# geo-ant/varpro

Measured on AMD Instinct MI355X. Metric: independent fits/sec (double-exp, m=1024, fp64), higher is better.
Workload: dtype f64; 1 GPU; B=65536 fits/GPU, m=1024, fp64, double-exp+offset (n=3, q=2), one full LM fit per step; batch_per_gpu=65536, m=1024, batches_in_flight=2, world_size=1, parallelism=batch-sharded x1

## Files before the change

bindings/rust/varpro_hip.rs:

```rust
#![allow(non_camel_case_types)]
use std::ffi::{c_char, c_void, CStr};
use std::ptr::null_mut;

use levenberg_marquardt::LeastSquaresProblem;
use nalgebra::storage::Owned;
use nalgebra::{DMatrix, DVector, Dyn};
use varpro::model::SeparableNonlinearModel;

#[repr(C)]
#[derive(Clone, Copy)]
pub struct vp_model_desc {
    pub n_basis: i32,
    pub n_params: i32,
    pub kind: [i32; 8],
    pub param: [[i32; 2]; 8],
}
#[repr(C)]
#[derive(Clone, Copy)]
pub struct vp_lm_opts {
    pub ftol: f64,
    pub xtol: f64,
    pub gtol: f64,
    pub stepbound: f64,
    pub patience: i32,
    pub scale_diag: i32,
}
#[repr(C)]
#[derive(Clone, Copy, Default)]
pub struct vp_report {
    pub termination: i32,
    pub n_evals: i32,
    pub objective: f64,
}
pub enum vp_batch {}

pub const VP_BASIS_CONST: i32 = 0;
pub const VP_BASIS_EXP_DECAY: i32 = 1;
pub const VP_BASIS_EXP_RATE: i32 = 2;
pub const VP_BASIS_EXP_COS: i32 = 3;
pub const VP_BASIS_SIN_PHASE: i32 = 4;
pub const VP_F64: i32 = 0;
pub const VP_FLAG_OWN_STREAM: i32 = 8;
pub const VP_FLAG_NO_GRID_RECURRENCE: i32 = 16;

#[link(name = "varpro_hip")]
extern "C" {
    pub fn vp_batch_create(h: *mut *mut vp_batch, model: *const vp_model_desc, dtype: i32, m: i64, s: i64, b: i64,
        t: *const c_void, y: *const c_void, w: *const c_void, svd_epsilon: f64, flags: i32, device: i32,
        hip_stream: *mut c_void) -> i32;
    pub fn vp_batch_destroy(h: *mut vp_batch);
    pub fn vp_set_params(h: *mut vp_batch, alpha: *const c_void) -> i32;
    pub fn vp_params(h: *mut vp_batch, alpha_out: *mut c_void) -> i32;
    pub fn vp_residuals(h: *mut vp_batch, r_out: *mut c_void, status: *mut i32) -> i32;
    pub fn vp_jacobian(h: *mut vp_batch, j_out: *mut c_void, status: *mut i32) -> i32;
    pub fn vp_linear_coeffs(h: *mut vp_batch, c_out: *mut c_void, status: *mut i32) -> i32;
    pub fn vp_weighted_data(h: *mut vp_batch, yw_out: *mut c_void) -> i32;
    pub fn vp_set_observations(h: *mut vp_batch, y: *const c_void) -> i32;
    pub fn vp_cost(h: *mut vp_batch, cost_out: *mut f64) -> i32;
    pub fn vp_evaluate(h: *mut vp_batch, alpha: *const c_void, r: *mut c_void, j: *mut c_void, c: *mut c_void,
        cost: *mut f64, status: *mut i32) -> i32;
    pub fn vp_basis(h: *mut vp_batch, alpha: *const c_void, phi: *mut c_void, dphi: *mut c_void, flags: i32) -> i32;
    pub fn vp_lm_opts_default(o: *mut vp_lm_opts, dtype: i32);
    pub fn vp_fit(h: *mut vp_batch, opts: *const vp_lm_opts, alpha_inout: *mut c_void, c_out: *mut c_void,
        rep: *mut vp_report) -> i32;
    pub fn vp_best_fit(h: *mut vp_batch, fit_out: *mut c_void) -> i32;
    pub fn vp_debug_gram_evaluate(h: *mut vp_batch, alpha: *const c_void, out: *mut f64) -> i32;
    pub fn vp_summary(h: *mut vp_batch, out: *mut f64) -> i32;
    pub fn vp_summary_device(h: *mut vp_batch, dev_out4: *mut f64) -> i32;
    pub fn vp_global_fit_condition(h: *mut vp_batch, cond_out: *mut f64) -> i32;
    pub fn vp_fit_trace(h: *mut vp_batch, opts: *const vp_lm_opts, alpha_inout: *mut c_void, c_out: *mut c_void,
        rep: *mut vp_report, trace_out: *mut f64, trace_rows: i32) -> i32;
    pub fn vp_statistics(h: *mut vp_batch, cov_out: *mut c_void, chi2_out: *mut f64, sigma_out: *mut c_void,
        status: *mut i32) -> i32;
    pub fn vp_global_statistics(h: *mut vp_batch, cov_alpha_out: *mut c_void, chi2_out: *mut f64, coef_cov_out: *mut c_void,
        coef_alpha_cov_out: *mut c_void, sigma_out: *mut c_void, status: *mut i32) -> i32;
    pub fn vp_set_rhs_allreduce(h: *mut vp_batch,
        f: Option<extern "C" fn(*mut c_void, i64, *mut c_void, *mut c_void) -> i32>, user: *mut c_void,
        global_rhs_count: i64) -> i32;
    pub fn vp_set_fit_kernel(h: *mut vp_batch, which: i32) -> i32;
    pub fn vp_set_timing(h: *mut vp_batch, enable: i32) -> i32;
    pub fn vp_last_kernel_ms(h: *mut vp_batch, which: i32, ms: *mut f32) -> i32;
    pub fn vp_synchronize(h: *mut vp_batch) -> i32;
    pub fn vp_last_error_detail() -> i32;
    pub fn vp_version() -> *const c_char;
    pub fn vp_device_count() -> i32;
    pub fn vp_last_error() -> *const c_char;
}

fn last_error() -> String {
    unsafe { CStr::from_ptr(vp_last_error()).to_string_lossy().into_owned() }
}

pub struct GpuSeparableProblem {
    h: *mut vp_batch,
    m: usize,
    s: usize,
    n: usize,
    q: usize,
    alpha: DVector<f64>,
}

impl GpuSeparableProblem {
    pub fn build(desc: vp_model_desc, x: &DVector<f64>, y: &DMatrix<f64>, w: Option<&DVector<f64>>, eps: Option<f64>,
                 initial: DVector<f64>) -> Result<Self, String> {
        let (m, s) = (y.nrows(), y.ncols());
        let mut h: *mut vp_batch = null_mut();
        let rc = unsafe {
            vp_batch_create(&mut h, &desc, VP_F64, m as i64, s as i64, 1, x.as_ptr() as *const c_void,
                y.as_ptr() as *const c_void, w.map_or(std::ptr::null(), |w| w.as_ptr() as *const c_void),
                eps.unwrap_or(-1.0), VP_FLAG_OWN_STREAM, 0, null_mut())
        };
        if rc != 0 { return Err(last_error()); }
        let mut p = Self { h, m, s, n: desc.n_basis as usize, q: desc.n_params as usize, alpha: initial.clone() };
        p.set_params(&initial);
        Ok(p)
    }
    pub fn linear_coefficients(&self) -> Option<DMatrix<f64>> {
// ... 155 lines not shown
```

include/varpro_hip.h:

```cpp
#ifndef VARPRO_HIP_H
#define VARPRO_HIP_H

#include <stdint.h>

#ifdef __cplusplus
extern "C" {
#endif

#define VP_MAX_BASIS 8
#define VP_MAX_PARAMS 8
#define VP_MAX_BASIS_PARAMS 2
#define VP_MAX_PAIRS 16

enum { VP_F64 = 0, VP_F32 = 1 };

enum {
    VP_BASIS_CONST = 0,
    VP_BASIS_EXP_DECAY = 1,
    VP_BASIS_EXP_RATE = 2,
    VP_BASIS_EXP_COS = 3,
    VP_BASIS_SIN_PHASE = 4,
    VP_BASIS_EXTERNAL = 5
};

// ... 70 lines not shown
typedef struct vp_batch vp_batch;


int vp_batch_create(vp_batch **h, const vp_model_desc *model, int dtype, int64_t m, int64_t S, int64_t B,
                    const void *t, const void *Y, const void *w, double svd_epsilon, int flags, int device,
                    void *hip_stream);

void vp_batch_destroy(vp_batch *h);


int vp_set_params(vp_batch *h, const void *alpha);

int vp_params(vp_batch *h, void *alpha_out);

int vp_residuals(vp_batch *h, void *r_out, int32_t *status);

int vp_jacobian(vp_batch *h, void *J_out, int32_t *status);

int vp_linear_coeffs(vp_batch *h, void *C_out, int32_t *status);

int vp_weighted_data(vp_batch *h, void *Yw_out);

int vp_set_observations(vp_batch *h, const void *Y);

int vp_cost(vp_batch *h, double *cost_out);

int vp_evaluate(vp_batch *h, const void *alpha, void *r_out, void *J_out, void *C_out, double *cost_out,
                int32_t *status);


enum { VP_BASIS_SKIP_INVARIANT = 1 };
int vp_basis(vp_batch *h, const void *alpha, void *Phi_out, void *dPhi_out, int flags);

int vp_batch_create_external(vp_batch **h, int32_t n_basis, int32_t n_params, int32_t n_pairs, const int32_t *pair_basis,
                             const int32_t *pair_param, int dtype, int64_t m, int64_t S, int64_t B, const void *Y,
                             const void *w, double svd_epsilon, int flags, int device, void *hip_stream);
int vp_set_params_with_basis(vp_batch *h, const void *alpha, const void *Phi, const void *dPhi);
int vp_jacobian_with_derivatives(vp_batch *h, const void *dPhi, void *J_out, int32_t *status);
int vp_evaluate_with_basis(vp_batch *h, const void *alpha, const void *Phi, const void *dPhi, void *r_out, void *J_out,
                           void *C_out, double *cost_out, int32_t *status);


void vp_lm_opts_default(vp_lm_opts *opts, int dtype);

enum { VP_FIT_DERIVATIVES_ON_ACCEPT = 1 };
enum { VP_WANT_BASIS = 1, VP_WANT_DERIVATIVES = 2 };
int vp_fit_begin(vp_batch *h, const vp_lm_opts *opts, const void *alpha0, int flags);
int vp_fit_step_with_basis(vp_batch *h, const void *Phi, const void *dPhi, void *alpha_trial_out, int32_t *want_out,
                           int64_t *n_active_out);
int vp_fit_end(vp_batch *h, void *alpha_out, void *C_out, vp_report *rep);
int vp_fit_active_set(vp_batch *h, int32_t *index_out, int32_t *count_out);

int vp_fit(vp_batch *h, const vp_lm_opts *opts, void *alpha_inout, void *C_out, vp_report *rep);

int vp_fit_trace(vp_batch *h, const vp_lm_opts *opts, void *alpha_inout, void *C_out, vp_report *rep,
                 double *trace_out, int trace_rows);

int vp_best_fit(vp_batch *h, void *fit_out);

int vp_statistics(vp_batch *h, void *cov_out, double *reduced_chi2_out, void *conf_sigma_out, int32_t *status);

int vp_global_statistics(vp_batch *h, void *cov_alpha_out, double *reduced_chi2_out, void *coef_cov_out,
                         void *coef_alpha_cov_out, void *conf_sigma_out, int32_t *status);

int vp_summary(vp_batch *h, double out[4]);

int vp_global_fit_condition(vp_batch *h, double *cond_out);

int vp_summary_device(vp_batch *h, double *dev_out4);

int vp_reduce_cost(vp_batch *h, void *rccl_comm, double out[4]);

typedef int (*vp_allreduce_fn)(void *dev_doubles, int64_t count, void *hip_stream, void *user);
int vp_set_rhs_allreduce(vp_batch *h, vp_allreduce_fn fn, void *user, int64_t global_rhs_count);

enum { VP_FIT_KERNEL_AUTO = 0, VP_FIT_KERNEL_WAVE = 1, VP_FIT_KERNEL_SLOTS = 2 };
int vp_set_fit_kernel(vp_batch *h, int which);


enum { VP_KERNEL_EVALUATE = 0, VP_KERNEL_BASIS = 1, VP_KERNEL_FIT = 2 };
int vp_set_timing(vp_batch *h, int enable);
int vp_last_kernel_ms(vp_batch *h, int which, float *ms);

int vp_synchronize(vp_batch *h);
const char *vp_last_error(void);
int vp_last_error_detail(void);
const char *vp_version(void);
int vp_device_count(void);

#ifdef __cplusplus
}
#endif
#endif
```

varpro_amd/_lib.py:

```python
import ctypes as C
import os

try:
    import torch
except Exception:
    torch = None

VP_MAX_BASIS = 8
VP_MAX_PARAMS = 8
VP_MAX_BASIS_PARAMS = 2
VP_MAX_PAIRS = 16

VP_F64, VP_F32 = 0, 1
VP_FLAG_DEVICE_PTRS, VP_FLAG_T_PER_PROBLEM, VP_FLAG_W_PER_PROBLEM, VP_FLAG_OWN_STREAM = 1, 2, 4, 8
VP_FLAG_NO_GRID_RECURRENCE = 16
VP_FLAG_STREAM_ROWS = 32
VP_BASIS_SKIP_INVARIANT = 1
VP_FIT_DERIVATIVES_ON_ACCEPT = 1
VP_WANT_BASIS, VP_WANT_DERIVATIVES = 1, 2
VP_KERNEL_EVALUATE, VP_KERNEL_BASIS, VP_KERNEL_FIT = 0, 1, 2
VP_ST_OK, VP_ST_NONFINITE, VP_ST_NOT_EVALUATED = 0, 1, 2

VP_ERR_OK, VP_ERR_INVALID, VP_ERR_UNSUPPORTED, VP_ERR_HIP, VP_ERR_NO_DEVICE = 0, -1, -2, -3, -4

_HERE = os.path.dirname(os.path.abspath(__file__))
LIB_PATH = os.path.join(_HERE, "lib", "libvarpro_hip.so")
if os.environ.get("VARPRO_HIP_LIBRARY"):
    LIB_PATH = os.path.abspath(os.environ["VARPRO_HIP_LIBRARY"])

ALLREDUCE_FN = C.CFUNCTYPE(C.c_int, C.c_void_p, C.c_int64, C.c_void_p, C.c_void_p)

VP_FIT_KERNEL_AUTO, VP_FIT_KERNEL_WAVE, VP_FIT_KERNEL_SLOTS = 0, 1, 2

ABI_SYMBOLS = [
    "vp_batch_create", "vp_batch_destroy", "vp_set_params", "vp_params", "vp_residuals", "vp_jacobian",
    "vp_linear_coeffs", "vp_weighted_data", "vp_set_observations", "vp_cost", "vp_evaluate", "vp_basis", "vp_lm_opts_default", "vp_fit", "vp_fit_trace",
    "vp_best_fit", "vp_statistics", "vp_summary", "vp_summary_device", "vp_global_fit_condition", "vp_set_rhs_allreduce", "vp_set_fit_kernel", "vp_set_timing", "vp_last_kernel_ms", "vp_synchronize", "vp_last_error",
    "vp_last_error_detail", "vp_version", "vp_device_count",
    "vp_batch_create_external", "vp_set_params_with_basis", "vp_jacobian_with_derivatives", "vp_evaluate_with_basis",
    "vp_reduce_cost", "vp_fit_begin", "vp_fit_step_with_basis", "vp_fit_end", "vp_fit_active_set", "vp_global_statistics",
]


DEBUG_SYMBOLS = ["vp_debug_gram_evaluate", "vp_debug_lmpar_gram", "vp_debug_set_refit"]


class VarproHipUnavailable(ImportError):
    pass


class VarproHipError(RuntimeError):
    def __init__(self, code, message, detail=0):
        super().__init__("varpro_hip error %d: %s" % (code, message))
        self.code = code
        self.detail = detail


class ModelDesc(C.Structure):
    _fields_ = [
        ("n_basis", C.c_int32),
        ("n_params", C.c_int32),
        ("kind", C.c_int32 * VP_MAX_BASIS),
        ("param", (C.c_int32 * VP_MAX_BASIS_PARAMS) * VP_MAX_BASIS),
    ]


class LmOpts(C.Structure):
    _fields_ = [
        ("ftol", C.c_double),
        ("xtol", C.c_double),
        ("gtol", C.c_double),
        ("stepbound", C.c_double),
        ("patience", C.c_int32),
        ("scale_diag", C.c_int32),
    ]


class Report(C.Structure):
    _fields_ = [("termination", C.c_int32), ("n_evals", C.c_int32), ("objective", C.c_double)]


_lib = None


def load():
    global _lib
    if _lib is not None:
        return _lib
    if not os.path.exists(LIB_PATH):
        raise VarproHipUnavailable(
            "%s not found: build it with `python -c 'import __graft_entry__ as g; g.build()'` "
            "(or `make -C varpro_amd/csrc`). varpro_amd has no CPU fallback." % LIB_PATH)
    try:
        lib = C.CDLL(LIB_PATH)
    except OSError as e:
        raise VarproHipUnavailable("cannot load %s: %s" % (LIB_PATH, e))
    vp, i32p, dp = C.c_void_p, C.POINTER(C.c_int32), C.POINTER(C.c_double)
    lib.vp_batch_create.argtypes = [C.POINTER(vp), C.POINTER(ModelDesc), C.c_int, C.c_int64, C.c_int64, C.c_int64,
                                    vp, vp, vp, C.c_double, C.c_int, C.c_int, vp]
    lib.vp_batch_create_external.argtypes = [C.POINTER(vp), C.c_int32, C.c_int32, C.c_int32, i32p, i32p, C.c_int, C.c_int64,
                                             C.c_int64, C.c_int64, vp, vp, C.c_double, C.c_int, C.c_int, vp]
    lib.vp_set_params_with_basis.argtypes = [vp, vp, vp, vp]
    lib.vp_jacobian_with_derivatives.argtypes = [vp, vp, vp, vp]
    lib.vp_evaluate_with_basis.argtypes = [vp, vp, vp, vp, vp, vp, vp, vp, vp]
    lib.vp_fit_begin.argtypes = [vp, C.POINTER(LmOpts), vp, C.c_int]
    lib.vp_fit_step_with_basis.argtypes = [vp, vp, vp, vp, vp, C.POINTER(C.c_int64)]
    lib.vp_fit_end.argtypes = [vp, vp, vp, vp]
    lib.vp_fit_active_set.argtypes = [vp, vp, vp]
    lib.vp_batch_destroy.argtypes = [vp]
    lib.vp_batch_destroy.restype = None
    lib.vp_set_params.argtypes = [vp, vp]
    lib.vp_set_observations.argtypes = [vp, vp]
    lib.vp_params.argtypes = [vp, vp]
    lib.vp_residuals.argtypes = [vp, vp, vp]
    lib.vp_jacobian.argtypes = [vp, vp, vp]
    lib.vp_linear_coeffs.argtypes = [vp, vp, vp]
    lib.vp_weighted_data.argtypes = [vp, vp]
    lib.vp_cost.argtypes = [vp, vp]
    lib.vp_evaluate.argtypes = [vp, vp, vp, vp, vp, vp, vp]
    lib.vp_basis.argtypes = [vp, vp, vp, vp, C.c_int]
    lib.vp_lm_opts_default.argtypes = [C.POINTER(LmOpts), C.c_int]
    lib.vp_lm_opts_default.restype = None
    lib.vp_fit.argtypes = [vp, C.POINTER(LmOpts), vp, vp, vp]
    lib.vp_fit_trace.argtypes = [vp, C.POINTER(LmOpts), vp, vp, vp, vp, C.c_int]
    lib.vp_best_fit.argtypes = [vp, vp]
    lib.vp_debug_gram_evaluate.argtypes = [vp, vp, vp]
    lib.vp_debug_lmpar_gram.argtypes = [C.c_int64, C.c_int, vp, vp, vp, vp, vp, vp, vp]
    lib.vp_debug_set_refit.argtypes = [vp, C.c_int]
    lib.vp_statistics.argtypes = [vp, vp, vp, vp, vp]
    lib.vp_global_statistics.argtypes = [vp, vp, vp, vp, vp, vp, vp]
    lib.vp_summary.argtypes = [vp, dp]
    lib.vp_summary_device.argtypes = [vp, vp]
    lib.vp_global_fit_condition.argtypes = [vp, vp]
    lib.vp_reduce_cost.argtypes = [vp, vp, dp]
    lib.vp_set_rhs_allreduce.argtypes = [vp, ALLREDUCE_FN, vp, C.c_int64]
    lib.vp_set_fit_kernel.argtypes = [vp, C.c_int]
    lib.vp_set_timing.argtypes = [vp, C.c_int]
    lib.vp_last_kernel_ms.argtypes = [vp, C.c_int, C.POINTER(C.c_float)]
    lib.vp_synchronize.argtypes = [vp]
    lib.vp_last_error.restype = C.c_char_p
    lib.vp_last_error_detail.restype = C.c_int
    lib.vp_version.restype = C.c_char_p
    lib.vp_device_count.restype = C.c_int
    _ = i32p
    _lib = lib
    return lib


def check(rc):
    if rc != 0:
        lib = load()
        raise VarproHipError(rc, lib.vp_last_error().decode("utf-8", "replace"), lib.vp_last_error_detail())


def device_count():
    return load().vp_device_count()
```

varpro_amd/batch.py:

```python
import ctypes as C

import numpy as np

from . import _lib
from ._lib import check

try:
    import torch
except Exception:
    torch = None

REPORT_DTYPE = np.dtype([("termination", np.int32), ("n_evals", np.int32), ("objective", np.float64)])

STATUS_OK, STATUS_NONFINITE, STATUS_NOT_EVALUATED = 0, 1, 2


def _is_torch(a):
    return torch is not None and isinstance(a, torch.Tensor)


class LevenbergMarquardt:

    def __init__(self, dtype=np.float64):
        eps = float(np.finfo(dtype).eps)
# ... 274 lines not shown
        J = self._empty((self.B, self.q, self.S * self.m))
        st = self._empty((self.B,), np.int32)
        check(self.lib.vp_jacobian(self._h, self._ptr(J), self._ptr(st)))
        if not self._have_params:
            J = None
        return (J, st) if with_status else J

    @_device_entry
    def linear_coefficients(self):
        Cm = self._empty((self.B, self.S, self.n))
        check(self.lib.vp_linear_coeffs(self._h, self._ptr(Cm), None))
        return Cm.reshape(self.B, self.n) if self.single_rhs else Cm

    @_device_entry
    def weighted_data(self):
        Yw = self._empty((self.B, self.S, self.m))
        check(self.lib.vp_weighted_data(self._h, self._ptr(Yw)))
        return Yw.reshape(self.B, self.m) if self.single_rhs else Yw

    @_device_entry
    def cost(self):
        c = self._empty((self.B,), np.float64)
        check(self.lib.vp_cost(self._h, self._ptr(c)))
        return c

    @_device_entry
    def evaluate(self, alpha, want_residuals=True, want_jacobian=True):
        a = self._as_array(alpha).reshape(self.B, self.q)
        r = self._empty((self.B, self.S * self.m)) if want_residuals else None
        J = self._empty((self.B, self.q, self.S * self.m)) if want_jacobian else None
        Cm = self._empty((self.B, self.S, self.n))
        cost = self._empty((self.B,), np.float64)
        st = self._empty((self.B,), np.int32)
        check(self.lib.vp_evaluate(self._h, self._ptr(a), self._ptr(r), self._ptr(J), self._ptr(Cm), self._ptr(cost),
                                   self._ptr(st)))
        self._have_params = True
        return dict(r=r, J=J, C=Cm.reshape(self.B, self.n) if self.single_rhs else Cm, cost=cost, status=st)

    @_device_entry
    def basis(self, alpha, skip_invariant=False, want_phi=True, want_dphi=True, out_phi=None, out_dphi=None):
        a = self._as_array(alpha).reshape(self.B, self.q)
        ncols = self.n - (sum(1 for k in self.model.kinds if k == 0) if skip_invariant else 0)
        phi = out_phi if out_phi is not None else (self._empty((self.B, ncols, self.m)) if want_phi else None)
        dphi = out_dphi if out_dphi is not None else (self._empty((self.B, self.p, self.m)) if want_dphi else None)
        check(self.lib.vp_basis(self._h, self._ptr(a), self._ptr(phi), self._ptr(dphi),
                                _lib.VP_BASIS_SKIP_INVARIANT if skip_invariant else 0))
        return phi, dphi

    @_device_entry
    def fit(self, alpha0, solver=None, want_coefficients=True):
        solver = solver or LevenbergMarquardt(self.np_dtype)
        opts = solver._c()
        a = self._as_array(alpha0).reshape(self.B, self.q)
        a = a.clone() if _is_torch(a) else a.copy()
        Cm = self._empty((self.B, self.S, self.n)) if want_coefficients else None
        if self.device_mode:
            rep_t = torch.empty((self.B, 16), dtype=torch.uint8, device=self._torch_device())
            check(self.lib.vp_fit(self._h, C.byref(opts), self._ptr(a), self._ptr(Cm), self._ptr(rep_t)))
            self._have_params = True
            rep = rep_t
            if Cm is not None and self.single_rhs:
                Cm = Cm.reshape(self.B, self.n)
            return a, Cm, rep
        else:
            rep = np.zeros(self.B, dtype=REPORT_DTYPE)
            check(self.lib.vp_fit(self._h, C.byref(opts), self._ptr(a), self._ptr(Cm), C.c_void_p(rep.ctypes.data)))
            self._have_params = True
        if Cm is not None and self.single_rhs:
            Cm = Cm.reshape(self.B, self.n)
        return a, Cm, rep

    @_device_entry
    def fit_begin(self, alpha0, solver=None, derivatives_on_accept=False):
        solver = solver or LevenbergMarquardt(self.np_dtype)
        opts = solver._c()
        a = self._as_array(alpha0).reshape(self.B, self.q)
        flags = _lib.VP_FIT_DERIVATIVES_ON_ACCEPT if derivatives_on_accept else 0
        check(self.lib.vp_fit_begin(self._h, C.byref(opts), self._ptr(a), flags))
        self._have_params = False
        self._xf_trial = self._empty((self.B, self.q))
        self._xf_want = self._empty((self.B,), np.int32)

    @_device_entry
    def fit_step_with_basis(self, Phi, dPhi=None, want_count=True):
        Phi = self._as_array(Phi).reshape(self.B, self.n, self.m)
        dPhi = None if dPhi is None else self._as_array(dPhi).reshape(self.B, self.p, self.m)
        self._ext_keep = (Phi, dPhi)
        nact = C.c_int64(0)
        check(self.lib.vp_fit_step_with_basis(self._h, self._ptr(Phi), self._ptr(dPhi), self._ptr(self._xf_trial),
                                              self._ptr(self._xf_want), C.byref(nact) if want_count else None))
        return self._xf_trial, self._xf_want, (int(nact.value) if want_count else None)

    @_device_entry
    def fit_active_set(self, index_out=None, count_out=None):
        idx = index_out if index_out is not None else self._empty((self.B,), np.int32)
        cnt = count_out if count_out is not None else self._empty((1,), np.int32)
        check(self.lib.vp_fit_active_set(self._h, self._ptr(idx), self._ptr(cnt)))
        return idx, cnt

    @_device_entry
    def fit_end(self, want_coefficients=True):
        a = self._empty((self.B, self.q))
        Cm = self._empty((self.B, self.n) if self.single_rhs else (self.B, self.S, self.n)) if want_coefficients else None
        if self.device_mode:
            rep = torch.empty((self.B, 16), dtype=torch.uint8, device=self._torch_device())
            check(self.lib.vp_fit_end(self._h, self._ptr(a), self._ptr(Cm), self._ptr(rep)))
        else:
            rep = np.zeros(self.B, dtype=REPORT_DTYPE)
            check(self.lib.vp_fit_end(self._h, self._ptr(a), self._ptr(Cm), C.c_void_p(rep.ctypes.data)))
        self._have_params = True
        return a, Cm, rep

    def fit_with_model(self, evaluate, alpha0, solver=None, derivatives_on_accept=False, max_steps=None, check_every=1):
        self.fit_begin(alpha0, solver, derivatives_on_accept)
        solver = solver or LevenbergMarquardt(self.np_dtype)
        limit = max_steps if max_steps is not None else 2 * (solver.patience * (self.q + 1) + 2)
        alpha, want = self._as_array(alpha0).reshape(self.B, self.q), None
# ... 156 lines not shown
```

varpro_amd/cpp/varpro.hpp:

```cpp
#pragma once
#include <algorithm>
#include <cmath>
#include <cstdint>
#include <functional>
#include <map>
#include <memory>
#include <optional>
#include <stdexcept>
#include <string>
#include <utility>
#include <vector>

#include "../../include/varpro_hip.h"

namespace varpro {

enum class Basis : int32_t {
    Const = VP_BASIS_CONST,
    ExpDecay = VP_BASIS_EXP_DECAY,
    ExpRate = VP_BASIS_EXP_RATE,
    ExpCos = VP_BASIS_EXP_COS,
    SinPhase = VP_BASIS_SIN_PHASE
};
inline int arity(Basis k) {
// ... 238 lines not shown
        n = model.desc.n_basis;
        q = model.desc.n_params;
        if ((int64_t)Y.size() != B * S * m) throw std::invalid_argument("Y must hold B*S*m values");
        check(vp_batch_create(&h_, &model.desc, VP_F64, m, S, B, model.x.data(), Y.data(), weights ? weights->data() : nullptr,
                              epsilon, VP_FLAG_OWN_STREAM, device, nullptr));
    }
    BatchProblem(const BatchProblem &) = delete;
    BatchProblem &operator=(const BatchProblem &) = delete;
    BatchProblem(BatchProblem &&o) noexcept { *this = std::move(o); }
    BatchProblem &operator=(BatchProblem &&o) noexcept {
        std::swap(h_, o.h_);
        m = o.m, S = o.S, B = o.B, n = o.n, q = o.q;
        return *this;
    }
    ~BatchProblem() {
        if (h_) vp_batch_destroy(h_);
    }
    vp_batch *handle() const { return h_; }
    void set_params(const std::vector<double> &alpha) { check(vp_set_params(h_, alpha.data())); }
    void set_observations(const std::vector<double> &Y) {
        if ((int64_t)Y.size() != B * S * m) throw std::invalid_argument("Y must hold B*S*m values");
        check(vp_set_observations(h_, Y.data()));
    }
    std::vector<int32_t> status() const {
        std::vector<int32_t> st((size_t)B);
        check(vp_linear_coeffs(h_, nullptr, st.data()));
        return st;
    }
    std::vector<double> residuals() const {
        std::vector<double> r((size_t)(B * S * m));
        check(vp_residuals(h_, r.data(), nullptr));
        return r;
    }
    std::vector<double> jacobian() const {
        std::vector<double> J((size_t)(B * q * S * m));
        check(vp_jacobian(h_, J.data(), nullptr));
        return J;
    }
    std::vector<double> linear_coefficients() const {
        std::vector<double> C((size_t)(B * S * n));
        check(vp_linear_coeffs(h_, C.data(), nullptr));
        return C;
    }
    std::vector<double> best_fit() const {
        std::vector<double> f((size_t)(B * S * m));
        check(vp_best_fit(h_, f.data()));
        return f;
    }
    std::vector<vp_report> fit(std::vector<double> &alpha_inout, const LevenbergMarquardt &solver = LevenbergMarquardt()) {
        std::vector<vp_report> rep((size_t)B);
        check(vp_fit(h_, &solver.o, alpha_inout.data(), nullptr, rep.data()));
        return rep;
    }
    struct Statistics {
        std::vector<double> covariance;
        std::vector<double> reduced_chi2;
        std::vector<double> conf_sigma;
        std::vector<int32_t> status;
        int64_t m = 0, dof = 0;
        std::vector<double> confidence_band_radius(int64_t b, double probability) const {
            if (!(probability > 0.0 && probability < 1.0)) throw std::invalid_argument("probability must be in (0,1)");
            const double tq = student_t_quantile(0.5 * (1.0 + probability), (double)dof);
            std::vector<double> r((size_t)m);
            for (int64_t i = 0; i < m; ++i) r[(size_t)i] = tq * conf_sigma[(size_t)(b * m + i)];
            return r;
        }
    };
    Statistics statistics() const {
        Statistics s;
        const size_t k = (size_t)(n + q);
        s.covariance.resize((size_t)B * k * k);
        s.reduced_chi2.resize((size_t)B);
        s.conf_sigma.resize((size_t)(B * m));
        s.status.resize((size_t)B);
        s.m = m;
        s.dof = m - (int64_t)k;
        check(vp_statistics(h_, s.covariance.data(), s.reduced_chi2.data(), s.conf_sigma.data(), s.status.data()));
        return s;
    }
    struct GlobalStatistics {
        std::vector<double> cov_alpha;
        std::vector<double> reduced_chi2;
        std::vector<double> coef_cov;
        std::vector<double> coef_alpha_cov;
        std::vector<double> conf_sigma;
        std::vector<int32_t> status;
        int64_t m = 0, S = 1, dof = 0;
        std::vector<double> confidence_band_radius(int64_t b, int64_t s, double probability) const {
            if (!(probability > 0.0 && probability < 1.0)) throw std::invalid_argument("probability must be in (0,1)");
            if (conf_sigma.empty()) throw std::logic_error("global_statistics(true) computes the band");
            const double tq = student_t_quantile(0.5 * (1.0 + probability), (double)dof);
            std::vector<double> r((size_t)m);
            for (int64_t i = 0; i < m; ++i) r[(size_t)i] = tq * conf_sigma[(size_t)((b * S + s) * m + i)];
            return r;
        }
    };
    GlobalStatistics global_statistics(bool want_confidence_sigma = false) const {
        GlobalStatistics g;
        g.cov_alpha.resize((size_t)(B * q * q));
        g.reduced_chi2.resize((size_t)B);
        g.coef_cov.resize((size_t)(B * S * n * n));
        g.coef_alpha_cov.resize((size_t)(B * S * n * q));
        if (want_confidence_sigma) g.conf_sigma.resize((size_t)(B * S * m));
        g.status.resize((size_t)B);
        g.m = m;
        g.S = S;
// ... 300 lines not shown
```

varpro_amd/csrc/vp_api.hip:

```cpp
#include <hip/hip_runtime.h>

#include <dlfcn.h>

#include <cfloat>
#include <cmath>
#include <cstdio>
#include <cstdlib>
#include <cstring>
#include <string>

#include "../../include/varpro_hip.h"
#include "../../include/varpro_hip_debug.h"
#include "vp_registry.hpp"
#include "vp_extfit_api.hpp"
#include "vp_mrhs.hpp"
#include "vp_gstats.hpp"

using namespace vp;

#ifndef VP_MRHS_EXACT_AFTER
#define VP_MRHS_EXACT_AFTER 8
#endif

namespace {
// ... 18 lines not shown

template <typename T>
__global__ void weight_data_kernel(const T *Y, const T *__restrict__ w, T *Yw, int m, int64_t cols_per_problem,
                                   int64_t w_stride, int64_t total) {
    for (int64_t idx = blockIdx.x * (int64_t)blockDim.x + threadIdx.x; idx < total;
         idx += (int64_t)gridDim.x * blockDim.x) {
        const int64_t col = idx / m;
        const int i = (int)(idx - col * m);
        const int64_t b = col / cols_per_problem;
        Yw[idx] = w ? (T)(w[b * w_stride + i] * Y[idx]) : Y[idx];
    }
}

__global__ void reduce_rhs_kernel(const double *__restrict__ cost_bs, const int32_t *__restrict__ status_bs,
                                  double *__restrict__ cost_b, int32_t *__restrict__ status_b, int S, int64_t B) {
    const int64_t b = blockIdx.x;
    if (b >= B) return;
    double acc = 0.0;
    int st = 0;
    for (int s0 = threadIdx.x; s0 < S; s0 += 8 * blockDim.x) {
        double c[8];
        int v[8];
#pragma unroll
        for (int k = 0; k < 8; ++k) {
            const int s = s0 + k * (int)blockDim.x;
            const bool in = s < S;
            c[k] = in ? cost_bs[b * S + s] : 0.0;
            v[k] = in ? status_bs[b * S + s] : 0;
        }
#pragma unroll
        for (int k = 0; k < 8; ++k) {
            acc += c[k];
            st = v[k] > st ? v[k] : st;
        }
    }
    __shared__ double sh[1024];
    __shared__ int shs[1024];
    sh[threadIdx.x] = acc;
    shs[threadIdx.x] = st;
    __syncthreads();
    for (int off = blockDim.x / 2; off > 0; off >>= 1) {
        if ((int)threadIdx.x < off) {
            sh[threadIdx.x] += sh[threadIdx.x + off];
            shs[threadIdx.x] = shs[threadIdx.x] > shs[threadIdx.x + off] ? shs[threadIdx.x] : shs[threadIdx.x + off];
        }
        __syncthreads();
    }
    if (threadIdx.x == 0) {
        if (cost_b) cost_b[b] = sh[0];
        if (status_b) status_b[b] = shs[0];
    }
}

__global__ void summary_kernel(const vp_report *__restrict__ rep, int64_t B, double *__restrict__ out4) {
    double c = 0, ok = 0, bad = 0, ev = 0;
    for (int64_t b = blockIdx.x * (int64_t)blockDim.x + threadIdx.x; b < B; b += (int64_t)gridDim.x * blockDim.x) {
        const vp_report r = rep[b];
        if (r.objective == r.objective) c += r.objective;
        if (r.termination > 0) ok += 1.0;
        else bad += 1.0;
        ev += (double)r.n_evals;
    }
    __shared__ double sh[4][256];
    sh[0][threadIdx.x] = c;
    sh[1][threadIdx.x] = ok;
    sh[2][threadIdx.x] = bad;
    sh[3][threadIdx.x] = ev;
    __syncthreads();
    for (int off = blockDim.x / 2; off > 0; off >>= 1) {
        if ((int)threadIdx.x < off)
            for (int k = 0; k < 4; ++k) sh[k][threadIdx.x] += sh[k][threadIdx.x + off];
        __syncthreads();
    }
    if (threadIdx.x == 0)
        for (int k = 0; k < 4; ++k) atomicAdd(&out4[k], sh[k][0]);
}

__global__ void mrhs_reduce_partials_kernel(const double *part, int gx, int nacc, int64_t B, double *tot) {
    const int64_t idx = blockIdx.x * (int64_t)blockDim.x + threadIdx.x;
    if (idx >= B * nacc) return;
    const int64_t b = idx / nacc;
    const int i = (int)(idx - b * nacc);
    double s = 0.0;
    for (int g = 0; g < gx; ++g) s += part[((size_t)b * nacc + i) * gx + g];
    tot[idx] = s;
}

template <typename T> __global__ void grid_check_kernel(const T *t, int m, int64_t ngrids, int *flag) {
    const int64_t g = blockIdx.x;
    if (g >= ngrids) return;
    const T *tg = t + g * (int64_t)m;
    const double t0 = (double)tg[0];
    const double dt = ((double)tg[m - 1] - t0) / (double)(m - 1);
    const double tol = 4.0 * (sizeof(T) == 8 ? 2.220446049250313e-16 : 1.1920928955078125e-07);
    bool ok = (dt == dt) && (dt - dt == 0.0) && dt != 0.0;
    for (int i = threadIdx.x; i < m; i += blockDim.x) {
        const double lat = __builtin_fma((double)i, dt, t0);
        const double dev = __builtin_fabs((double)tg[i] - lat);
        if (!(dev <= tol * __builtin_fabs((double)tg[i] - t0))) ok = false;
    }
    if (!ok) atomicAnd(flag, 0);
}

}

struct vp_batch {
    vp_model_desc model;
    int dtype;
    int64_t m, S, B;
    int n, q, p;
    int flags;
    int device;
    double eps;
    hipStream_t stream;
    bool own_stream;
    const KernelEntry *kern;
    void *d_t, *d_w, *d_yw;
    void *d_alpha;
    void *d_C;
    void *d_R;
    double *d_cost_bs;
    int32_t *d_status_bs;
    double *d_cost;
    int32_t *d_status;
    vp_report *d_report;
    double *d_sum4;
    bool grid_uniform;
    bool have_params;
    bool r_valid;
    bool have_report;
    bool timing;
    hipEvent_t ev0, ev1;
    float last_ms[3];
    bool have_mrhs;
    MrhsWs mrhs;
    vp_allreduce_fn rhs_allreduce;
    void *rhs_allreduce_user;
    int64_t rhs_global;
    double *d_mrhs_tot;
    void *d_gen_lm;
    int32_t *d_gen_nactive;
    int fit_kernel;
    int *d_queue;
    int num_cus;
    void *tmp_a, *tmp_b;
    void *d_gen_ws;
    int gen_blocks;
    int64_t m_user;
    hipGraphExec_t mrhs_graph;
    hipGraphExec_t mrhs_graph_tail;
    bool external;
    int ext_np;
    int32_t ext_pb[VP_MAX_PAIRS], ext_pp[VP_MAX_PAIRS];
    const void *ext_phi, *ext_dphi;
    void *ext_phi_own, *ext_dphi_own;
    int mrhs_graph_len;
    int mrhs_graph_iters;
    int mrhs_prev_nfev;
    int mrhs_same_count;
    int32_t *h_nactive;
    int32_t *h_nactive_dev;
    MrhsIo *h_io;
    MrhsIo *h_io_dev;
    vp_lm_opts mrhs_graph_opts;
    hipStream_t cap_stream;
    bool mrhs_graph_failed;
    void *d_xf_state;
    void *d_xf_trial;
    int32_t *d_xf_want;
    void *d_xf_ctrial;
    int32_t *d_xf_active;
    int64_t xf_known_active;
    int32_t *d_xf_nactive;
    int32_t *h_xf_nactive;
    bool xf_running;
    bool xf_init;
    int xf_flags;
    int64_t xf_steps;
    vp_lm_opts xf_opts;
    int32_t *d_rescue;
    void *d_rescue_ws;
    int rescue_slot;
    bool rescue_off;
};

namespace {

bool device_ptrs(const vp_batch *h) { return (h->flags & VP_FLAG_DEVICE_PTRS) != 0; }

struct InBuf {
    const void *dptr = nullptr;
    void *tmp = nullptr;
    int init(vp_batch *h, const void *user, size_t bytes) {
        if (!user) {
            dptr = nullptr;
// ... 206 lines not shown
    return 0;
}

int run_evaluate(vp_batch *h, void *r_dev, void *J_dev, void *C_dev) {
    if (h->external && !h->ext_phi)
        return fail(VP_ERR_INVALID, "the columns of the handle's current parameters are not known (after vp_fit_end: call "
                                    "vp_set_params_with_basis with Phi / dPhi at the fitted parameters first)");
    if (h->external && !h->d_gen_ws &&
        !external_resident(h->dtype, h->n, h->ext_np, h->m, h->m_user ? h->m_user : h->m, J_dev != nullptr))
        if (int rc = ensure_gen_ws(h)) return rc;
    LaunchParams p;
    fill_params(h, p);
    p.r_out = r_dev;
    p.J_out = J_dev;
    p.C_out = C_dev;
    p.cost_out = h->d_cost_bs;
    p.status = h->d_status_bs;
    Timer tm(h, VP_KERNEL_EVALUATE);
    int rc;
    if (h->have_mrhs) {
        p.mrhs_ws = &h->mrhs;
        p.mrhs_mode = 1;
        rc = h->kern->mrhs_factor(p);
        if (rc == VP_ERR_OK) rc = h->kern->mrhs_stream(p);
    } else {
        rc = h->kern->evaluate(p);
    }
    tm.stop();
    if (rc != VP_ERR_OK) return fail(rc, "evaluate kernel launch failed");
    return reduce_rhs(h);
}

struct DeviceGuard {
    int prev = -1;
    bool armed = false;
    int enter(int device) {
        if (hipGetDevice(&prev) != hipSuccess) prev = -1;
        if (prev != device) {
            VP_HIP(hipSetDevice(device));
            armed = prev >= 0;
        }
        return 0;
    }
    ~DeviceGuard() {
        if (armed) (void)hipSetDevice(prev);
    }
};

#define VP_ENTER(h)                                                                                                   \
    if (!(h)) return fail(VP_ERR_INVALID, "null handle");                                                             \
    DeviceGuard dev_guard__;                                                                                          \
    if (int rc__ = dev_guard__.enter((h)->device)) return rc__

int mrhs_fit(vp_batch *h, const vp_lm_opts *opts, void *alpha_inout, void *C_out, vp_report *rep, double *trace_out,
             int trace_rows) {
    if (!h->have_mrhs && !h->kern->mrhs_fit_whole) return fail(VP_ERR_UNSUPPORTED, "no MRHS kernels for this (model, m)");
    vp_lm_opts o;
    if (opts) o = *opts;
    else vp_lm_opts_default(&o, h->dtype);
    const size_t ts = tsize(h->dtype);
    const hipMemcpyKind kin = device_ptrs(h) ? hipMemcpyDeviceToDevice : hipMemcpyHostToDevice;
    const bool use_io = device_ptrs(h) && h->have_mrhs;
    if (!h->h_nactive) {
        VP_HIP(hipHostMalloc((void **)&h->h_nactive, 2 * sizeof(int32_t), hipHostMallocMapped));
        VP_HIP(hipHostGetDevicePointer((void **)&h->h_nactive_dev, h->h_nactive, 0));
        VP_HIP(hipHostMalloc((void **)&h->h_io, sizeof(MrhsIo), hipHostMallocMapped));
        VP_HIP(hipHostGetDevicePointer((void **)&h->h_io_dev, h->h_io, 0));
        std::memset(h->h_io, 0, sizeof(MrhsIo));
    }
    if (use_io) {
        h->h_io->alpha_in = alpha_inout;
        h->h_io->alpha_out = alpha_inout;
        h->h_io->C_out = C_out;
        h->h_io->rep_out = rep;
    } else {
        std::memset(h->h_io, 0, sizeof(MrhsIo));
        VP_HIP(hipMemcpyAsync(h->d_alpha, alpha_inout, (size_t)h->B * h->q * ts, kin, h->stream));
    }
    LaunchParams p;
    fill_params(h, p);
    p.mrhs_ws = &h->mrhs;
    p.opts = &o;
    OutBuf tr;
    const size_t tr_bytes = (size_t)h->B * (size_t)(trace_rows > 0 ? trace_rows : 0) * (h->q + 4) * sizeof(double);
    if (trace_out && trace_rows > 0) {
        if (int rc = tr.init(h, trace_out, tr_bytes)) return rc;
        VP_HIP(hipMemsetAsync(tr.dptr, 0xFF, tr_bytes, h->stream));
        p.trace = (double *)tr.dptr;
        p.trace_rows = trace_rows;
    }
    if (!h->have_mrhs) {
        p.alpha_out = h->d_alpha;
        p.C_out = h->d_C;
        p.cost_out = h->d_cost_bs;
        p.status = h->d_status_bs;
        p.report = h->d_report;
        if (h->rhs_allreduce) {
            const int nacc = 2 + h->q * h->q + h->q;
            if (!h->d_gen_lm) VP_HIP(hipMalloc(&h->d_gen_lm, (size_t)h->B * h->kern->mrhs_state_bytes));
            if (!h->d_mrhs_tot) VP_HIP(hipMalloc((void **)&h->d_mrhs_tot, (size_t)h->B * nacc * sizeof(double)));
            if (!h->d_gen_nactive) VP_HIP(hipMalloc((void **)&h->d_gen_nactive, sizeof(int32_t)));
            VP_HIP(hipMemsetAsync(h->d_gen_nactive, 0, sizeof(int32_t), h->stream));
            p.gen_lm_state = h->d_gen_lm;
            p.gen_acc = h->d_mrhs_tot;
            p.gen_nactive = h->d_gen_nactive;
            p.mrhs_S_global = h->rhs_global;
            Timer tm(h, VP_KERNEL_FIT);
            p.gen_phase = 1;
            if (int rc = h->kern->mrhs_fit_whole(p)) return fail(rc, "generic global-fit (init) launch failed");
            const int max_iter = o.patience * (h->q + 1) + 2;
            for (int it = 0; it < max_iter; ++it) {
                p.gen_phase = 2;
                if (int rc = h->kern->mrhs_fit_whole(p)) return fail(rc, "generic global-fit (sums) launch failed");
                if (h->rhs_allreduce(h->d_mrhs_tot, h->B * nacc, (void *)h->stream, h->rhs_allreduce_user) != 0)
                    return fail(VP_ERR_INVALID, "the right-hand-side all-reduce callback reported an error");
                p.gen_phase = 3;
                if (int rc = h->kern->mrhs_fit_whole(p)) return fail(rc, "generic global-fit (step) launch failed");
                if ((it & 3) == 3 || it + 1 == max_iter) {
                    int32_t nact = 0;
                    VP_HIP(hipMemcpyAsync(&nact, h->d_gen_nactive, sizeof(int32_t), hipMemcpyDeviceToHost, h->stream));
                    VP_HIP(hipStreamSynchronize(h->stream));
                    if (nact <= 0) break;
                }
            }
            p.gen_phase = 4;
            if (int rc = h->kern->mrhs_fit_whole(p)) return fail(rc, "generic global-fit (results) launch failed");
            tm.stop();
        } else {
            Timer tm(h, VP_KERNEL_FIT);
            if (int rc = h->kern->mrhs_fit_whole(p)) return fail(rc, "generic global-fit launch failed");
// ... 409 lines not shown
    if (try_uniform) {
        const int one = 1;
        VP_TRY(hipMalloc((void **)&d_gflag, sizeof(int)));
        VP_TRY(hipMemcpyAsync(d_gflag, &one, sizeof(int), hipMemcpyHostToDevice, h->stream));
        const int64_t ngrids = (flags & VP_FLAG_T_PER_PROBLEM) ? B : 1;
        if (dtype == VP_F64)
            hipLaunchKernelGGL(grid_check_kernel<double>, dim3((unsigned)ngrids), dim3(256), 0, h->stream,
                               (const double *)h->d_t, (int)m, ngrids, d_gflag);
        else
            hipLaunchKernelGGL(grid_check_kernel<float>, dim3((unsigned)ngrids), dim3(256), 0, h->stream,
                               (const float *)h->d_t, (int)m, ngrids, d_gflag);
        VP_TRY(hipGetLastError());
    }
    VP_TRY(hipMalloc(&h->d_yw, y_elems * ts));
    {
        void *&ytmp = h->tmp_b;
        const void *ysrc = Y;
        if (!data_on_device) {
            VP_TRY(hipMalloc(&ytmp, y_elems * ts));
            VP_TRY(hipMemcpyAsync(ytmp, Y, y_elems * ts, hipMemcpyHostToDevice, h->stream));
            ysrc = ytmp;
        }
        const int64_t total = (int64_t)y_elems;
        const unsigned grid = (unsigned)std::min<int64_t>((total + 255) / 256, 65536);
        const int64_t wstride = (flags & VP_FLAG_W_PER_PROBLEM) ? m : 0;
        if (dtype == VP_F64)
            hipLaunchKernelGGL(weight_data_kernel<double>, dim3(grid), dim3(256), 0, h->stream, (const double *)ysrc,
                               (const double *)h->d_w, (double *)h->d_yw, (int)m, S, wstride, total);
        else
            hipLaunchKernelGGL(weight_data_kernel<float>, dim3(grid), dim3(256), 0, h->stream, (const float *)ysrc,
                               (const float *)h->d_w, (float *)h->d_yw, (int)m, S, wstride, total);
        VP_TRY(hipGetLastError());
        int gflag = 0;
        if (d_gflag) VP_TRY(hipMemcpyAsync(&gflag, d_gflag, sizeof(int), hipMemcpyDeviceToHost, h->stream));
        VP_TRY(hipStreamSynchronize(h->stream));
        (void)hipFree(ytmp);
        ytmp = nullptr;
        (void)hipFree(d_gflag);
        d_gflag = nullptr;
        h->grid_uniform = gflag != 0;
    }
    VP_TRY(hipMalloc(&h->d_alpha, (size_t)std::max<int64_t>(1, B * h->q) * ts));
    VP_TRY(hipMalloc(&h->d_C, (size_t)B * S * h->n * ts));
    VP_TRY(hipMalloc((void **)&h->d_cost_bs, (size_t)B * S * sizeof(double)));
    VP_TRY(hipMalloc((void **)&h->d_status_bs, (size_t)B * S * sizeof(int32_t)));
    if (S == 1) {
        h->d_cost = h->d_cost_bs;
        h->d_status = h->d_status_bs;
    } else {
        VP_TRY(hipMalloc((void **)&h->d_cost, (size_t)B * sizeof(double)));
        VP_TRY(hipMalloc((void **)&h->d_status, (size_t)B * sizeof(int32_t)));
    }
    VP_TRY(hipMalloc((void **)&h->d_report, (size_t)B * sizeof(vp_report)));
    VP_TRY(hipMalloc((void **)&h->d_sum4, 4 * sizeof(double)));
    VP_TRY(hipMalloc((void **)&h->d_queue, sizeof(int)));
    if (kern->uses_gen_ws && !ext) {
        if (int rc = ensure_gen_ws(h)) {
            vp_batch_destroy(h);
            return rc;
        }
    }
    VP_TRY(hipEventCreate(&h->ev0));
    VP_TRY(hipEventCreate(&h->ev1));
    if (S > 1 && kern->mrhs_factor && kern->mrhs_stream && kern->mrhs_lm && kern->mrhs_finish) {
        const int n_ = h->n, p_ = h->p, q_ = h->q;
        VP_TRY(hipMalloc(&h->mrhs.qthin, (size_t)B * n_ * m * ts));
        VP_TRY(hipMalloc(&h->mrhs.g, (size_t)B * std::max(1, p_) * m * ts));
        VP_TRY(hipMalloc((void **)&h->mrhs.small, (size_t)B * mrhs_small_stride_rt(n_, p_) * sizeof(double)));
        VP_TRY(hipMalloc((void **)&h->mrhs.statusA, (size_t)B * sizeof(int32_t)));
        const int gx_acc = mrhs_gx(S, kern->mrhs_gx_cap > 0 ? kern->mrhs_gx_cap : 256);
        if (gx_acc > VP_MRHS_GX_MAX) {
            vp_batch_destroy(h);
            return fail(VP_ERR_INVALID, "internal: partial-sum slots per problem exceed VP_MRHS_GX_MAX");
        }
        VP_TRY(hipMalloc((void **)&h->mrhs.acc, (size_t)B * gx_acc * (1 + n_ * n_ + p_) * sizeof(double)));
        VP_TRY(hipMalloc(&h->mrhs.lm_state, (size_t)B * kern->mrhs_state_bytes));
        VP_TRY(hipMalloc((void **)&h->mrhs.nactive, 2 * sizeof(int32_t)));
        VP_TRY(hipMalloc((void **)&h->mrhs.done, (size_t)B * sizeof(int32_t)));
        VP_TRY(hipMemsetAsync(h->mrhs.done, 0, (size_t)B * sizeof(int32_t), h->stream));
        VP_TRY(hipMalloc(&h->mrhs.alpha_trial, (size_t)std::max<int64_t>(1, B * q_) * ts));
        for (int i = 0; i < 2; ++i) {
            VP_TRY(hipMalloc(&h->mrhs.cbuf[i], (size_t)B * S * n_ * ts));
            VP_TRY(hipMalloc((void **)&h->mrhs.costbuf[i], (size_t)B * S * sizeof(double)));
            VP_TRY(hipMalloc((void **)&h->mrhs.stbuf[i], (size_t)B * S * sizeof(int32_t)));
        }
        VP_TRY(hipMalloc((void **)&h->mrhs.widx, (size_t)B * sizeof(int32_t)));
        VP_TRY(hipMalloc((void **)&h->mrhs.bidx, (size_t)B * sizeof(int32_t)));
        VP_TRY(hipMalloc((void **)&h->mrhs.jcond, (size_t)B * sizeof(double)));
        VP_TRY(hipMemsetAsync(h->mrhs.jcond, 0, (size_t)B * sizeof(double), h->stream));
        h->have_mrhs = true;
    }
#undef VP_TRY
    for (int k = 0; k < 3; ++k) h->last_ms[k] = -1.f;
    *out = h;
    return VP_ERR_OK;
}

void vp_batch_destroy(vp_batch *h) {
    if (!h) return;
    DeviceGuard dev_guard__;
    (void)dev_guard__.enter(h->device);
    (void)hipStreamSynchronize(h->stream);
    (void)hipFree(h->d_mrhs_tot);
    (void)hipFree(h->d_gen_lm);
    (void)hipFree(h->d_gen_nactive);
    (void)hipFree(h->d_t);
    (void)hipFree(h->d_w);
    (void)hipFree(h->d_yw);
// ... 398 lines not shown
    return copy_out(h, cost_out, h->d_cost, (size_t)h->B * sizeof(double));
}

int vp_evaluate(vp_batch *h, const void *alpha, void *r_out, void *J_out, void *C_out, double *cost_out,
                int32_t *status) {
    VP_ENTER(h);
    VP_NOT_EXTERNAL(h, "vp_evaluate");
    if (!alpha) return fail(VP_ERR_INVALID, "null alpha");
    const size_t ts = tsize(h->dtype);
    VP_HIP(hipMemcpyAsync(h->d_alpha, alpha, (size_t)h->B * h->q * ts,
                          device_ptrs(h) ? hipMemcpyDeviceToDevice : hipMemcpyHostToDevice, h->stream));
    RowOut r, J;
    if (int rc = r.init(h, r_out, (size_t)h->B * h->S)) return rc;
    if (int rc = J.init(h, J_out, (size_t)h->B * h->q * h->S)) return rc;
    if (int rc = run_evaluate(h, r.dptr, J.dptr, h->d_C)) return rc;
    h->have_params = true;
    h->r_valid = false;
    if (int rc = r.finish(h)) return rc;
    if (int rc = J.finish(h)) return rc;
    if (int rc = copy_out(h, C_out, h->d_C, (size_t)h->B * h->S * h->n * ts)) return rc;
    if (int rc = copy_out(h, cost_out, h->d_cost, (size_t)h->B * sizeof(double))) return rc;
    return copy_status(h, status);
}

int vp_basis(vp_batch *h, const void *alpha, void *Phi_out, void *dPhi_out, int flags) {
    VP_ENTER(h);
    VP_NOT_EXTERNAL(h, "vp_basis");
    if (!alpha) return fail(VP_ERR_INVALID, "null alpha");
    const size_t ts = tsize(h->dtype);
    int ncols = 0;
    for (int j = 0; j < h->n; ++j)
        if (!((flags & VP_BASIS_SKIP_INVARIANT) && h->model.kind[j] == VP_BASIS_CONST)) ++ncols;
    InBuf a;
    if (int rc = a.init(h, alpha, (size_t)h->B * h->q * ts)) return rc;
    RowOut phi, dphi;
    if (int rc = phi.init(h, Phi_out, (size_t)h->B * ncols)) return rc;
    if (int rc = dphi.init(h, dPhi_out, (size_t)h->B * h->p)) return rc;
    LaunchParams p;
    fill_params(h, p);
    p.alpha = a.dptr;
    p.Phi_out = phi.dptr;
    p.dPhi_out = dphi.dptr;
    p.basis_flags = flags;
    Timer tm(h, VP_KERNEL_BASIS);
    int rc = h->kern->basis(p);
    tm.stop();
    if (rc != VP_ERR_OK) return fail(rc, "basis kernel launch failed");
    if (int rc2 = phi.finish(h)) return rc2;
    if (int rc2 = dphi.finish(h)) return rc2;
    if (!device_ptrs(h)) VP_HIP(hipStreamSynchronize(h->stream));
    return VP_ERR_OK;
}

int vp_fit(vp_batch *h, const vp_lm_opts *opts, void *alpha_inout, void *C_out, vp_report *rep) {
    return vp_fit_trace(h, opts, alpha_inout, C_out, rep, nullptr, 0);
}

namespace {
constexpr int kRescueBlocks = 8;
int rescue_prepare(vp_batch *h, LaunchParams &p) {
    if (h->rescue_off || h->kern->family == FAMILY_GENERIC || h->kern->gram_fit) return 0;
    if (!h->d_rescue) {
        VP_HIP(hipMalloc((void **)&h->d_rescue, (size_t)(2 + h->B) * sizeof(int32_t)));
        VP_HIP(hipMemsetAsync(h->d_rescue, 0, 2 * sizeof(int32_t), h->stream));
        h->rescue_slot = 0;
    }
    if (!h->d_rescue_ws) {
        const size_t slot = (size_t)(h->n + 1 + h->p + h->q) * (size_t)h->m * tsize(h->dtype);
        VP_HIP(hipMalloc(&h->d_rescue_ws, (size_t)kRescueBlocks * slot));
    }
    p.rescue = h->d_rescue;
    p.rescue_slot = h->rescue_slot;
    return 0;
}
int rescue_refit(vp_batch *h, const LaunchParams &fit_params) {
    if (!fit_params.rescue) return 0;
    LaunchParams p = fit_params;
    p.gen_list_first = 0;
    if (launch_fn fast = find_fit_rescue(h->kern->fit_single)) {
        const int rc = fast(p);
        if (rc == VP_ERR_OK) p.gen_list_first = kFitRescueGrid;
        else if (rc != VP_ERR_UNSUPPORTED) return rc;
    }
    p.rescue = nullptr;
    p.gen_ws = h->d_rescue_ws;
    p.gen_blocks = kRescueBlocks;
    p.gen_list = h->d_rescue;
    p.gen_list_slot = h->rescue_slot;
    p.gen_scale_cols = 1;
    h->rescue_slot ^= 1;
    return generic_kernels(h->dtype)->fit_single(p);
}
}

int vp_fit_trace(vp_batch *h, const vp_lm_opts *opts, void *alpha_inout, void *C_out, vp_report *rep,
                 double *trace_out, int trace_rows) {
    VP_ENTER(h);
    VP_NOT_EXTERNAL(h, "vp_fit");
    if (!alpha_inout) return fail(VP_ERR_INVALID, "null alpha");
    if (h->m_user && (int64_t)h->q > h->m_user * h->S) {
        const size_t ts = tsize(h->dtype);
        VP_HIP(hipMemcpyAsync(h->d_alpha, alpha_inout, (size_t)h->B * h->q * ts,
                              device_ptrs(h) ? hipMemcpyDeviceToDevice : hipMemcpyHostToDevice, h->stream));
        if (int rc = run_evaluate(h, nullptr, nullptr, h->d_C)) return rc;
        OutBuf trw;
        if (trace_out && trace_rows > 0) {
            const size_t trb = (size_t)h->B * (size_t)trace_rows * (h->q + 4) * sizeof(double);
            if (int rc = trw.init(h, trace_out, trb)) return rc;
            VP_HIP(hipMemsetAsync(trw.dptr, 0xFF, trb, h->stream));
        }
        hipLaunchKernelGGL(wrong_dimensions_report_kernel, dim3((unsigned)((h->B + 255) / 256)), dim3(256), 0, h->stream,
                           (const double *)h->d_cost, (const int32_t *)h->d_status, h->B, h->d_report,
                           trw.dptr ? (double *)trw.dptr : nullptr, trace_rows, h->q, h->dtype, (const void *)h->d_alpha);
        VP_HIP(hipGetLastError());
        h->have_params = true;
        h->r_valid = false;
        h->have_report = true;
        if (int rc = copy_out(h, C_out, h->d_C, (size_t)h->B * h->S * h->n * ts)) return rc;
        if (int rc = copy_out(h, rep, h->d_report, (size_t)h->B * sizeof(vp_report))) return rc;
        return trw.finish(h);
    }
    if (h->S != 1) return mrhs_fit(h, opts, alpha_inout, C_out, rep, trace_out, trace_rows);
    if (!h->kern->fit && !h->kern->fit_single) return fail(VP_ERR_UNSUPPORTED, "no fit kernel for this model");
    vp_lm_opts o;
    if (opts) o = *opts;
    else vp_lm_opts_default(&o, h->dtype);
    const size_t ts = tsize(h->dtype);
    VP_HIP(hipMemcpyAsync(h->d_alpha, alpha_inout, (size_t)h->B * h->q * ts,
                          device_ptrs(h) ? hipMemcpyDeviceToDevice : hipMemcpyHostToDevice, h->stream));
    LaunchParams p;
    fill_params(h, p);
    p.alpha_out = h->d_alpha;
    p.C_out = h->d_C;
    p.cost_out = h->d_cost_bs;
    p.status = h->d_status_bs;
    p.report = h->d_report;
    p.opts = &o;
    OutBuf tr;
    const size_t tr_bytes = (size_t)h->B * (size_t)(trace_rows > 0 ? trace_rows : 0) * (h->q + 4) * sizeof(double);
    if (trace_out && trace_rows > 0) {
        if (int rc = tr.init(h, trace_out, tr_bytes)) return rc;
        VP_HIP(hipMemsetAsync(tr.dptr, 0xFF, tr_bytes, h->stream));
        p.trace = (double *)tr.dptr;
        p.trace_rows = trace_rows;
    }
    launch_fn fit_fn = h->kern->fit ? h->kern->fit : h->kern->fit_single;
    if (int rc0 = rescue_prepare(h, p)) return rc0;
    int list_used = 0;
    p.rescue_used = &list_used;
    Timer tm(h, VP_KERNEL_FIT);
    int rc = fit_fn(p);
    if (rc == VP_ERR_OK && list_used) rc = rescue_refit(h, p);
    tm.stop();
    if (rc != VP_ERR_OK) return fail(rc, "fit kernel launch failed");
    h->have_params = true;
    h->r_valid = false;
    h->have_report = true;
    if (int rc2 = copy_out(h, alpha_inout, h->d_alpha, (size_t)h->B * h->q * ts)) return rc2;
    if (int rc2 = copy_out(h, C_out, h->d_C, (size_t)h->B * h->n * ts)) return rc2;
    if (int rc2 = copy_out(h, rep, h->d_report, (size_t)h->B * sizeof(vp_report))) return rc2;
    if (int rc2 = tr.finish(h)) return rc2;
    return VP_ERR_OK;
}

int vp_debug_set_refit(vp_batch *h, int enabled) {
    VP_ENTER(h);
    h->rescue_off = enabled == 0;
    return VP_ERR_OK;
}

int vp_debug_gram_evaluate(vp_batch *h, const void *alpha, double *out) {
    VP_ENTER(h);
    if (!alpha || !out) return fail(VP_ERR_INVALID, "null argument");
    if (h->external || h->S != 1 || !h->kern->gram_fit || !h->kern->fit)
        return fail(VP_ERR_UNSUPPORTED, "the handle's fit does not run on the Gram kernel (fp32, exponentials + offset beyond one wavefront)");
    const size_t ts = tsize(h->dtype);
    const int per = 1 + h->n + h->q + h->q * h->q;
    InBuf a;
    if (int rc = a.init(h, alpha, (size_t)h->B * h->q * ts)) return rc;
    OutBuf o;
    if (int rc = o.init(h, out, (size_t)h->B * per * sizeof(double))) return rc;
    vp_lm_opts opt;
    vp_lm_opts_default(&opt, h->dtype);
    LaunchParams p;
    fill_params(h, p);
    p.alpha_out = const_cast<void *>(a.dptr);
    p.opts = &opt;
    p.gram_dbg = (double *)o.dptr;
    if (int rc = h->kern->fit(p)) return fail(rc, "Gram evaluation launch failed");
    return o.finish(h);
}

extern "C++" {
namespace {
template <int Q>
__global__ void debug_lmpar_gram_kernel(int64_t B, const double *Rj, const int32_t *ipvt, const double *diag, const double *qtb,
                                        const double *delta, const double *par_in, double *out) {
    const int64_t b = (int64_t)blockIdx.x * blockDim.x + threadIdx.x;
    if (b >= B) return;
    double r[Q][Q], dg[Q], qb[Q], step[Q];
    int ip[Q];
#pragma unroll
    for (int i = 0; i < Q; ++i) {
        dg[i] = diag[b * Q + i];
        qb[i] = qtb[b * Q + i];
        ip[i] = ipvt[b * Q + i];
        step[i] = 0.0;
#pragma unroll
        for (int j = 0; j < Q; ++j) r[i][j] = Rj[(b * Q + i) * Q + j];
    }
    double dxnorm = 0.0;
    const double par = vp::lmpar_chol<double, Q, false, (Q > 3)>(r, ip, dg, qb, delta[b], par_in[b], step, dxnorm);
    double *o = out + b * (Q + 2);
// ... 184 lines not shown
        st_dev = (int32_t *)st_tmp.p;
    }
    char *wsb = (char *)ws.p;
    void *basis_ws = h->external ? nullptr : wsb;
    gp.ws_cols = (double *)(wsb + sz_basis);
    gp.ws_rows = band ? (double *)(wsb + sz_basis + sz_cols) : nullptr;
    gp.ws_small = (double *)(wsb + sz_basis + sz_cols + sz_rows);
    const char *wdev = (const char *)h->d_w;
    for (int64_t b0 = 0; b0 < B; b0 += bc) {
        const int64_t nb = std::min<int64_t>(bc, B - b0);
        if (h->external) {
            gp.phi = (const char *)h->ext_phi + (size_t)b0 * n * gp.rows * ts;
            gp.dphi = h->ext_dphi ? (const char *)h->ext_dphi + (size_t)b0 * P * gp.rows * ts : nullptr;
        } else {
            LaunchParams p;
            fill_params(h, p);
            p.B = nb;
            p.alpha = (const char *)h->d_alpha + (size_t)b0 * q * ts;
            p.t = (const char *)h->d_t + (size_t)b0 * p.t_stride * ts;
            p.w = h->d_w ? wdev + (size_t)b0 * p.w_stride * ts : nullptr;
            p.Phi_out = basis_ws;
            p.dPhi_out = (char *)basis_ws + (size_t)nb * n * m * ts;
            p.basis_flags = 0;
            if (int rc = h->kern->basis(p)) return fail(rc, "basis kernel launch failed");
            gp.phi = p.Phi_out;
            gp.dphi = P > 0 ? p.dPhi_out : nullptr;
        }
        gp.B = nb;
        gp.w = h->d_w ? wdev + (size_t)b0 * gp.w_stride * ts : nullptr;
        gp.C = (const char *)h->d_C + (size_t)b0 * S * n * ts;
        gp.cost = h->d_cost + b0;
        gp.status_in = h->d_status + b0;
        gp.cov_alpha = (char *)cov.dptr + (size_t)b0 * q * q * ts;
        gp.chi2 = (double *)chi2.dptr + b0;
        gp.coef_cov = cc.dptr ? (char *)cc.dptr + (size_t)b0 * S * n * n * ts : nullptr;
        gp.coef_alpha_cov = ca.dptr ? (char *)ca.dptr + (size_t)b0 * S * n * q * ts : nullptr;
        gp.band = sig.dptr ? (char *)sig.dptr + (size_t)b0 * S * m * ts : nullptr;
        gp.status_out = st_dev + b0;
        if (int rc = gstats_launch(gp)) return fail(rc, "global statistics kernels failed");
    }
    if (int rc = cov.finish(h)) return rc;
    if (int rc = chi2.finish(h)) return rc;
    if (int rc = cc.finish(h)) return rc;
    if (int rc = ca.finish(h)) return rc;
    if (int rc = sig.finish(h)) return rc;
    if (status && !device_ptrs(h)) {
        VP_HIP(hipMemcpyAsync(status, st_dev, (size_t)B * sizeof(int32_t), hipMemcpyDeviceToHost, h->stream));
        VP_HIP(hipStreamSynchronize(h->stream));
    }
    if (device_ptrs(h)) VP_HIP(hipStreamSynchronize(h->stream));
    return VP_ERR_OK;
}

int vp_summary(vp_batch *h, double out[4]) {
    VP_ENTER(h);
    if (!h->have_report) return fail(VP_ERR_INVALID, "vp_summary requires a completed vp_fit");
    VP_HIP(hipMemsetAsync(h->d_sum4, 0, 4 * sizeof(double), h->stream));
    const unsigned grid = (unsigned)std::min<int64_t>((h->B + 255) / 256, 1024);
    hipLaunchKernelGGL(summary_kernel, dim3(grid), dim3(256), 0, h->stream, h->d_report, h->B, h->d_sum4);
    VP_HIP(hipGetLastError());
    VP_HIP(hipMemcpyAsync(out, h->d_sum4, 4 * sizeof(double), hipMemcpyDeviceToHost, h->stream));
    VP_HIP(hipStreamSynchronize(h->stream));
    return VP_ERR_OK;
}

int vp_global_fit_condition(vp_batch *h, double *cond_out) {
    VP_ENTER(h);
    if (!cond_out) return fail(VP_ERR_INVALID, "null output");
    if (!h->have_mrhs || !h->mrhs.jcond || !h->have_report)
        return fail(VP_ERR_INVALID, "vp_global_fit_condition requires a completed vp_fit on a handle with several right-hand sides "
                                    "(specialised kernel set)");
    return copy_out(h, cond_out, h->mrhs.jcond, (size_t)h->B * sizeof(double));
}

int vp_summary_device(vp_batch *h, double *dev_out4) {
    VP_ENTER(h);
    if (!h->have_report) return fail(VP_ERR_INVALID, "vp_summary_device requires a completed vp_fit");
    if (!dev_out4) return fail(VP_ERR_INVALID, "null output");
    VP_HIP(hipMemsetAsync(dev_out4, 0, 4 * sizeof(double), h->stream));
    const unsigned grid = (unsigned)std::min<int64_t>((h->B + 255) / 256, 1024);
    hipLaunchKernelGGL(summary_kernel, dim3(grid), dim3(256), 0, h->stream, h->d_report, h->B, dev_out4);
    VP_HIP(hipGetLastError());
    return VP_ERR_OK;
}

typedef int (*vp_nccl_allreduce_t)(const void *, void *, size_t, int, int, void *, hipStream_t);
static vp_nccl_allreduce_t resolve_nccl_allreduce() {
    static vp_nccl_allreduce_t fn = nullptr;
    static bool tried = false;
    if (!tried) {
        tried = true;
        void *sym = dlsym(RTLD_DEFAULT, "ncclAllReduce");
        if (!sym) {
            void *lib = dlopen("librccl.so.1", RTLD_NOW | RTLD_GLOBAL);
            if (!lib) lib = dlopen("librccl.so", RTLD_NOW | RTLD_GLOBAL);
            if (lib) sym = dlsym(lib, "ncclAllReduce");
        }
        fn = reinterpret_cast<vp_nccl_allreduce_t>(sym);
    }
    return fn;
}

int vp_reduce_cost(vp_batch *h, void *rccl_comm, double out[4]) {
    VP_ENTER(h);
    if (!out) return fail(VP_ERR_INVALID, "null output");
    if (!h->have_report) return fail(VP_ERR_INVALID, "vp_reduce_cost requires a completed vp_fit");
    VP_HIP(hipMemsetAsync(h->d_sum4, 0, 4 * sizeof(double), h->stream));
    const unsigned grid = (unsigned)std::min<int64_t>((h->B + 255) / 256, 1024);
    hipLaunchKernelGGL(summary_kernel, dim3(grid), dim3(256), 0, h->stream, h->d_report, h->B, h->d_sum4);
    VP_HIP(hipGetLastError());
    if (rccl_comm) {
        vp_nccl_allreduce_t ar = resolve_nccl_allreduce();
        if (!ar) return fail(VP_ERR_UNSUPPORTED, "ncclAllReduce not found: link librccl or make librccl.so.1 loadable");
        const int rc = ar(h->d_sum4, h->d_sum4, 4,  8,  0, rccl_comm, h->stream);
        if (rc != 0) return fail(VP_ERR_HIP, "ncclAllReduce failed with code " + std::to_string(rc));
    }
    VP_HIP(hipMemcpyAsync(out, h->d_sum4, 4 * sizeof(double), hipMemcpyDeviceToHost, h->stream));
    VP_HIP(hipStreamSynchronize(h->stream));
    return VP_ERR_OK;
}

int vp_set_fit_kernel(vp_batch *h, int which) {
    if (!h) return fail(VP_ERR_INVALID, "null handle");
    if (which != VP_FIT_KERNEL_AUTO && which != VP_FIT_KERNEL_WAVE && which != VP_FIT_KERNEL_SLOTS)
        return fail(VP_ERR_INVALID, "vp_set_fit_kernel: unknown kernel selector");
    h->fit_kernel = which;
    return VP_ERR_OK;
}

int vp_set_timing(vp_batch *h, int enable) {
    if (!h) return fail(VP_ERR_INVALID, "null handle");
    h->timing = enable != 0;
    return VP_ERR_OK;
}

int vp_last_kernel_ms(vp_batch *h, int which, float *ms) {
    if (!h || !ms || which < 0 || which > 2) return fail(VP_ERR_INVALID, "bad argument");
    *ms = h->last_ms[which];
    return VP_ERR_OK;
}

int vp_synchronize(vp_batch *h) {
    VP_ENTER(h);
    VP_HIP(hipStreamSynchronize(h->stream));
    return VP_ERR_OK;
}

}

namespace vp {

std::vector<RescueEntry> &rescue_registry() {
    static std::vector<RescueEntry> r;
    return r;
}
std::vector<KernelEntry> &registry() {
    static std::vector<KernelEntry> r;
    return r;
}

static int kind_arity(int kind) {
    switch (kind) {
    case VP_BASIS_CONST: return 0;
    case VP_BASIS_EXP_DECAY:
    case VP_BASIS_EXP_RATE: return 1;
    case VP_BASIS_EXP_COS:
    case VP_BASIS_SIN_PHASE: return 2;
    default: return -1;
    }
}

int classify_model(const vp_model_desc &d, int &a, int &b, int &c, int &p_out) {
    int pairs = 0;
    for (int j = 0; j < d.n_basis; ++j) {
        const int ar = kind_arity(d.kind[j]);
        if (ar < 0) return -1;
        for (int k = 0; k < VP_MAX_BASIS_PARAMS; ++k) {
            const int pi = d.param[j][k];
// ... 60 lines not shown
```

varpro_amd/csrc/vp_fit.hpp:

```cpp
#pragma once
#include "vp_kernels.hpp"

namespace vp {

template <bool U> __device__ __forceinline__ bool pol(bool c) {
    if constexpr (U) return uni(c);
    else return c;
}
template <bool U> __device__ __forceinline__ int pol(int v) {
    if constexpr (U) return uni(v);
    else return v;
}

template <typename T, int Q, bool U = true> __device__ __forceinline__ T enorm_small(const T (&v)[Q]) {
    T s = T(0);
#pragma unroll
    for (int j = 0; j < Q; ++j) s = tfma(v[j], v[j], s);
    if (pol<U>(s > T(1e-280) && s < T(1e280))) return usqrt(s);
    T mx = T(0);
#pragma unroll
    for (int j = 0; j < Q; ++j) mx = tmax(mx, tabs(v[j]));
    if (!(mx > T(0)) || !is_finite(mx)) return (s != s) ? s : mx;
    s = T(0);
    const T inv = T(1) / mx;
// ... 855 lines not shown
#pragma unroll
                    for (int r = 0; r < R; ++r) {
                        const T v = (r >= L::VW || L::row_of(r, lane) > prow) ? Z[k][r] : T(0);
                        s2 = tfma(v, v, s2);
                    }
                    rdiag[k] = tsqrt(group_sum(grp, s2));
                    wa[k] = rdiag[k];
                }
            }
        }
        {
            const T f = gj * tfma(an, top[NREM], dr);
#pragma unroll
            for (int r = 0; r < R; ++r) rv[r] = tfma(f, Z[j][r], rv[r]);
            qtf[j] = tfma(f, vp, top[NREM]);
        }
        rdiag[j] = -an;
    });
#pragma unroll
    for (int j = 0; j < Q; ++j) Rj[j][j] = sc[j] * rdiag[j];
}

template <typename T, int Q> __device__ __forceinline__ bool jac_not_finite(const T (&acnorm)[Q]) {
    bool bad = false;
#pragma unroll
    for (int k = 0; k < Q; ++k) bad = bad || !is_finite(acnorm[k]);
    return bad;
}

template <typename T, class M> struct FitArgs {
    M mdl;
    const T *t;
    const T *w;
    const T *yw;
    T *alpha;
    T *C_out;
    double *cost_out;
    int32_t *status;
    vp_report *report;
    int m;
    int64_t B;
    int64_t t_stride, w_stride;
    T eps;
    T ftol, xtol, gtol, stepbound;
    int patience;
    int scale_diag;
    double *trace;
    int trace_rows;
    int grid_uniform;
    int32_t *rescue;
    int rescue_slot;
};

template <typename T, int N, int Q> struct LmState {
    T x[Q], diag[Q], qtf[Q], acnorm[Q], cbest[N];
    T Rj[Q][Q];
    T fnorm, delta, par, xnorm, gnorm, pnorm, prered, dirder, objective;
    int ipvt[Q];
    int flags;
    int nfev;
};

template <typename T, class M> inline constexpr bool fit_rescue_v = M::kStatic && M::kConstLast && M::kDiagonalPairs;

template <typename T, class M, int R, int W, bool WEIGHTED, int PADM, bool RESCUE, bool SELF>
__device__ __forceinline__ bool fit_problem(const FitArgs<T, M> &a, const int64_t b, T *s_t, T *s_y, T *s_w, unsigned char *xch,
                                            LmState<T, M::N, M::Q> *st, const bool stage_grid) {
    static_assert(!(WEIGHTED && PADM != 0), "PADM is a unit-weight specialisation");
    static_assert(!RESCUE || fit_rescue_v<T, M>, "the scaled re-fit needs the constant-first sweep and diagonal pairs");
    constexpr int N = M::N, P = M::P, Q = M::Q;
    constexpr bool CF = M::kConstLast;
    constexpr int NC = CF ? N + P : N + 1 + P;
    constexpr int YC = CF ? N - 1 : N;
    constexpr int DC = YC + 1;
    constexpr int MP = 64 * R * W;
    using G = Grp<W>;
    G grp = G::make(xch);
    const int lane = grp.gl;
    const int m = a.m;

    {
        T tmp[R];
        if (stage_grid) {
            const T *tp = a.t + b * a.t_stride;
            load_rows<T, R, W>(tp, m, lane, vec_aligned<T>(tp, m), tmp);
            store_rows<T, R, W>(s_t, MP, lane, true, tmp);
        }
        if constexpr (WEIGHTED) {
            const T *wp = a.w + b * a.w_stride;
            load_rows<T, R, W>(wp, m, lane, vec_aligned<T>(wp, m), tmp);
            store_rows<T, R, W>(s_w, MP, lane, true, tmp);
        }
        const T *yp = a.yw + b * (int64_t)m;
        load_rows<T, R, W>(yp, m, lane, vec_aligned<T>(yp, m), tmp);
        store_rows<T, R, W>(s_y, MP, lane, true, tmp);
    }
    if constexpr (W > 1) {
        __syncthreads();
    } else {
        __builtin_amdgcn_wave_barrier();
        asm volatile("s_waitcnt lgkmcnt(0)" ::: "memory");
    }
    using Src = RowSource<T, R, true, WEIGHTED ? 1 : 0, 1, W, true, PADM>;
    Src src;
    src.t = s_t;
    src.w = s_w;
    src.m = m;
    src.lane = lane;
    src.vec = true;
    src.set_uniform(a.grid_uniform != 0);
    ConstReflector<T> h0;
    if constexpr (CF) h0 = make_const_reflector<T, R, Src, G>(src, grp);

    T x[Q], xt[Q], diag[Q], qtf[Q], step[Q], acnorm[Q], cbest[N];
    T Rj[Q][Q];
    int ipvt[Q];
#pragma unroll
    for (int k = 0; k < Q; ++k) {
        xt[k] = a.alpha[b * Q + k];
        x[k] = xt[k];
        diag[k] = T(1);
        qtf[k] = T(0);
        step[k] = T(0);
        acnorm[k] = T(0);
        ipvt[k] = k;
#pragma unroll
        for (int j = 0; j < Q; ++j) Rj[k][j] = T(0);
    }
#pragma unroll
    for (int k = 0; k < N; ++k) cbest[k] = T(0);
    T fnorm = T(0), delta = T(0), par = T(0), xnorm = T(0), gnorm = T(0);
    T pnorm = T(0), prered = T(0), dirder = T(0);
    T objective = T(0) / T(0);
    bool first = true, first_tr = true, first_update = true;
    int nfev = 0, term = VP_TERM_NOT_RUN;
    int st_best = VP_ST_NOT_EVALUATED;
    bool flagged = false;
    const int max_fev = a.patience * (Q + 1);
    const int mres = m;
    int trow = 0;
    auto trace_row = [&](const T(&xx)[Q], T fn, T ratio) {
        if (a.trace && trow < a.trace_rows && lane == 0) {
            double *tr = a.trace + ((size_t)b * a.trace_rows + trow) * (Q + 4);
#pragma unroll
            for (int k = 0; k < Q; ++k) tr[k] = (double)xx[k];
            tr[Q] = (double)fn;
            tr[Q + 1] = (double)ratio;
            tr[Q + 2] = (double)delta;
            tr[Q + 3] = (double)par;
        }
        ++trow;
    };

#ifdef VP_FIT_CLOCKS
    SectionClock clk_, *clk = &clk_;
    clk_.start();
#else
    SectionClock *clk = nullptr;
#endif
    auto park = [&]() __attribute__((always_inline)) {
        if (grp.lane == 0) {
#pragma unroll
            for (int k = 0; k < Q; ++k) {
                st->x[k] = x[k];
                st->diag[k] = diag[k];
                st->qtf[k] = qtf[k];
                st->acnorm[k] = acnorm[k];
                st->ipvt[k] = ipvt[k];
#pragma unroll
                for (int j = 0; j < Q; ++j) st->Rj[k][j] = Rj[k][j];
            }
#pragma unroll
// ... 221 lines not shown
#pragma unroll
                for (int k = 0; k < Q; ++k) diag[k] = tmax(diag[k], acnorm[k]);
            }
        }

        VP_TICK(clk, 6);
        par = lmpar_any<T, Q>(Rj, ipvt, diag, qtf, delta, par, step, pnorm);
        VP_TICK(clk, 7);
        if (uni(!is_finite(pnorm))) {
            term = VP_TERM_NUMERICAL;
            break;
        }
        {
            T wa[Q];
#pragma unroll
            for (int i = 0; i < Q; ++i) wa[i] = T(0);
#pragma unroll
            for (int j = 0; j < Q; ++j) {
                const T pj = dyn_get<Q>(step, ipvt[j]);
#pragma unroll
                for (int i = 0; i <= j; ++i) wa[i] = tfma(Rj[i][j], pj, wa[i]);
            }
            const T ifn = frcp(fnorm);
            const T t1 = enorm_small<T, Q>(wa) * ifn;
            const T temp1 = t1 * t1;
            const T t2 = (usqrt(par) * pnorm) * ifn;
            const T temp2 = t2 * t2;
            if (uni(!is_finite(temp1) || !is_finite(temp2))) {
                term = VP_TERM_NUMERICAL;
                break;
            }
            prered = temp1 + temp2 * T(2);
            dirder = -(temp1 + temp2);
        }
        if (first_tr && pnorm < delta) delta = pnorm;
        first_tr = false;
#pragma unroll
        for (int k = 0; k < Q; ++k) xt[k] = x[k] - step[k];
        VP_TICK(clk, 8);
    }
#ifdef VP_FIT_CLOCKS
    if (a.trace && lane == 0 && a.trace_rows * (Q + 4) >= 12) {
        double *tr = a.trace + (size_t)b * a.trace_rows * (Q + 4);
        for (int k = 0; k < 12; ++k) tr[k] = (double)clk_.acc[k];
    }
#endif

    if (lane == 0) {
        vp_report rep;
        rep.termination = term;
        rep.n_evals = nfev;
        rep.objective = (double)objective;
        a.report[b] = rep;
        if (a.cost_out) a.cost_out[b] = (double)objective;
        if (a.status) a.status[b] = st_best;
    }
    if (lane == 0) {
        if (flagged && (SELF || a.rescue != nullptr)) {
            if (!SELF) rescue_push(a.rescue, a.rescue_slot, b);
        } else {
#pragma unroll
            for (int k = 0; k < Q; ++k) a.alpha[b * Q + k] = x[k];
        }
        if (a.C_out) {
#pragma unroll
            for (int k = 0; k < N; ++k) a.C_out[b * N + a.mdl.out_index(k)] = cbest[k];
        }
    }
    return flagged;
}

template <typename T, class M, int R, int W, bool WEIGHTED, int PADM = 0, bool RESCUE = false>
__global__ void __launch_bounds__(64 * W, (model_waves_for<T, M, R, M::N + 1 + M::P>())) fit_kernel(const FitArgs<T, M> a) {
    constexpr int MP = 64 * R * W;
    extern __shared__ __attribute__((aligned(16))) unsigned char smem_raw[];
    T *s_t = reinterpret_cast<T *>(smem_raw);
    T *s_y = s_t + MP;
    T *s_w = WEIGHTED ? s_y + MP : nullptr;
    unsigned char *s_after = reinterpret_cast<unsigned char *>(s_y + MP + (WEIGHTED ? MP : 0));
    LmState<T, M::N, M::Q> *st = reinterpret_cast<LmState<T, M::N, M::Q> *>(s_after + ((group_xch_bytes<W>() + 15) / 16) * 16) +
                                 (W > 1 ? (int)(threadIdx.x >> 6) : 0);
    int64_t b = blockIdx.x;
    if constexpr (RESCUE) {
        if (b >= (int64_t)uni(a.rescue[a.rescue_slot])) return;
        b = (int64_t)uni(a.rescue[2 + b]);
    } else {
        if (b >= a.B) return;
    }
    (void)fit_problem<T, M, R, W, WEIGHTED, PADM, RESCUE, false>(a, b, s_t, s_y, s_w, s_after, st, true);
}

template <typename T, class M, int R, int W> constexpr size_t fit_lds_bytes(bool weighted) {
    return (size_t)(weighted ? 3 : 2) * 64 * R * W * sizeof(T) + ((group_xch_bytes<W>() + 15) / 16) * 16 +
           (size_t)W * sizeof(LmState<T, M::N, M::Q>);
}
template <typename T, class M, int R, int W = 1> int launch_fit(const LaunchParams &p) {
    FitArgs<T, M> a;
    if (!bind_model(*p.model, a.mdl)) return VP_ERR_UNSUPPORTED;
    sweep_invariant_first(a.mdl);
    a.t = (const T *)p.t;
    a.w = (const T *)p.w;
    a.yw = (const T *)p.yw;
    a.alpha = (T *)p.alpha_out;
    a.C_out = (T *)p.C_out;
    a.cost_out = p.cost_out;
    a.status = p.status;
    a.report = p.report;
    a.m = p.m;
    a.B = p.B;
    a.t_stride = p.t_stride;
    a.w_stride = p.w_stride;
    a.eps = (T)p.eps;
    a.ftol = (T)p.opts->ftol;
    a.xtol = (T)p.opts->xtol;
    a.gtol = (T)p.opts->gtol;
    a.stepbound = (T)p.opts->stepbound;
    a.patience = p.opts->patience;
    a.scale_diag = p.opts->scale_diag;
    a.trace = p.trace;
    a.trace_rows = p.trace_rows;
    a.grid_uniform = p.grid_uniform;
    a.rescue = p.rescue;
    a.rescue_slot = p.rescue_slot;
    if (a.B <= 0) return VP_ERR_OK;
    if (p.rescue_used) *p.rescue_used = 1;
    const size_t lds = fit_lds_bytes<T, M, R, W>(p.w != nullptr);
    if (p.w) hipLaunchKernelGGL((fit_kernel<T, M, R, W, true>), dim3((unsigned)a.B), dim3(64 * W), lds, p.stream, a);
    else if (p.m == 64 * R * W)
        hipLaunchKernelGGL((fit_kernel<T, M, R, W, false, 1>), dim3((unsigned)a.B), dim3(64 * W), lds, p.stream, a);
    else if (R > 2 && p.m > 64 * (R - 2) * W)
        hipLaunchKernelGGL((fit_kernel<T, M, R, W, false, 2>), dim3((unsigned)a.B), dim3(64 * W), lds, p.stream, a);
    else hipLaunchKernelGGL((fit_kernel<T, M, R, W, false>), dim3((unsigned)a.B), dim3(64 * W), lds, p.stream, a);
    return hipGetLastError() == hipSuccess ? VP_ERR_OK : VP_ERR_HIP;
}

template <typename T, class M, int R, int W = 1> int launch_fit_rescue(const LaunchParams &p) {
    if constexpr (!fit_rescue_v<T, M>) {
        return VP_ERR_UNSUPPORTED;
    } else {
        if (p.w || p.t_stride != 0 || !p.rescue) return VP_ERR_UNSUPPORTED;
        FitArgs<T, M> a;
        if (!bind_model(*p.model, a.mdl)) return VP_ERR_UNSUPPORTED;
        a.t = (const T *)p.t;
        a.w = nullptr;
        a.yw = (const T *)p.yw;
        a.alpha = (T *)p.alpha_out;
        a.C_out = (T *)p.C_out;
        a.cost_out = p.cost_out;
        a.status = p.status;
        a.report = p.report;
        a.m = p.m;
        a.B = p.B;
        a.t_stride = 0;
        a.w_stride = 0;
        a.eps = (T)p.eps;
        a.ftol = (T)p.opts->ftol;
        a.xtol = (T)p.opts->xtol;
        a.gtol = (T)p.opts->gtol;
        a.stepbound = (T)p.opts->stepbound;
        a.patience = p.opts->patience;
        a.scale_diag = p.opts->scale_diag;
        a.trace = p.trace;
        a.trace_rows = p.trace_rows;
        a.grid_uniform = p.grid_uniform;
        a.rescue = p.rescue;
        a.rescue_slot = p.rescue_slot;
        const size_t lds = fit_lds_bytes<T, M, R, W>(false);
        hipLaunchKernelGGL((fit_kernel<T, M, R, W, false, 0, true>), dim3(kFitRescueGrid), dim3(64 * W), lds, p.stream, a);
        return hipGetLastError() == hipSuccess ? VP_ERR_OK : VP_ERR_HIP;
    }
}

template <typename T, class M> struct BestFitArgs {
    M mdl;
    const T *t;
    const T *alpha;
    const T *C;
    T *out;
    int m, S;
    int64_t nprob;
    int64_t t_stride;
};

template <typename T, class M, int R, int W>
__global__ void __launch_bounds__(64 * W) best_fit_kernel(const BestFitArgs<T, M> a) {
    constexpr int N = M::N, P = M::P, Q = M::Q, NC = N + 1 + P;
    const int lane = (int)threadIdx.x;
    const int64_t prob = blockIdx.x;
    if (prob >= a.nprob) return;
    const int64_t b = prob / a.S;
    const int m = a.m;
    T alpha[Q], c[N];
#pragma unroll
    for (int k = 0; k < Q; ++k) alpha[k] = a.alpha[b * Q + k];
#pragma unroll
    for (int k = 0; k < N; ++k) c[k] = a.C[prob * N + k];
    using Src = RowSource<T, R, false, 0, 0, W>;
    Src src;
    src.t = a.t + b * a.t_stride;
    src.w = nullptr;
    src.m = m;
    src.lane = lane;
    src.vec = false;
    T C[NC][R];
    build_columns<T, M, R, NC, Src>(a.mdl, alpha, src, C);
    T f[R];
#pragma unroll
    for (int r = 0; r < R; ++r) {
        T acc = T(0);
#pragma unroll
        for (int j = 0; j < N; ++j) acc = tfma(C[j][r], c[j], acc);
        f[r] = acc;
    }
    T *op = a.out + prob * (int64_t)m;
    store_rows<T, R, W>(op, m, lane, vec_aligned<T>(op, m), f);
}

template <typename T, class M, int R, int W = 1> int launch_best_fit(const LaunchParams &p) {
    BestFitArgs<T, M> a;
    if (!bind_model(*p.model, a.mdl)) return VP_ERR_UNSUPPORTED;
    a.t = (const T *)p.t;
// ... 14 lines not shown
```

varpro_amd/csrc/vp_fit2.hpp:

```cpp
#pragma once
#include "vp_fit.hpp"

namespace vp {

template <typename T, int N, int Q> struct alignas(8) SlotRec {
    T xt[Q], x[Q], diag[Q], qtf[Q], acnorm[Q], cbest[N], cnew[N];
    T Rj[Q][Q];
    T fnorm, delta, par, xnorm, gnorm, pnorm, prered, dirder, objective;
    T fnorm1, actred, ratio;
    T qty0;
    T pre[2 * Q + 2];
    int ipvt[Q];
    int flags;
    int nfev;
    int term;
    int status;
    int prob;
    int trow;
    int pend[2];
};

#ifndef VP_FIT2_PRE
#define VP_FIT2_PRE 1
#endif
#ifndef VP_SLOT_CAP
#define VP_SLOT_CAP 8
#endif
template <typename T, int R, int W, int NG, int BLOCKS_PER_CU, int REC = 0> constexpr int fit2_slots() {
    constexpr int col = 64 * R * W * (int)sizeof(T);
    constexpr int budget = (160 * 1024) / BLOCKS_PER_CU - col - 3 * 1024;
    constexpr int gs = budget / (NG * (col + REC));
    return gs < 1 ? 1 : (gs > VP_SLOT_CAP ? VP_SLOT_CAP : gs);
}

#ifndef VP_FITG_TIMELINE
#define VP_FITG_TIMELINE 0
#endif
template <typename T, class M> struct Fit2Args {
    FitArgs<T, M> f;
    int *queue;
    int waves_total;
};


template <typename T, typename TO = T> struct SlotConsts {
    T ftol, xtol, gtol, stepbound;
    TO *alpha;
    TO *C_out;
    double *cost_out;
    int32_t *status;
    vp_report *report;
    double *trace;
    const TO *yw;
    int *queue;
    int32_t *rescue;
    int rescue_slot;
    int self_rescue;
    int64_t B;
    int trace_rows, scale_diag, max_fev, m;
    T eps;
    T pre_delta;
#ifdef VP_FIT2_CLOCKS
    long long sck[6];
#endif
};

template <typename T, int R, class Src, class G>
__device__ __forceinline__ T fill_slot_column(const T *__restrict__ yp, const int m, T *s_col, const Src &src,
                                              const ConstReflector<T> &h0, G &grp) {
    using L = Layout<R, G::W>;
    constexpr int VW = L::VW;
    const int lane = grp.gl;
    T y[R];
    load_rows<T, R, G::W>(yp, m, lane, vec_aligned<T>(yp, m), y);
    T acc = T(0);
#pragma unroll
    for (int r0 = 0; r0 < R; r0 += VW) {
        T tt[2], sc[2];
        src.get(r0, tt, sc);
#pragma unroll
        for (int e = 0; e < VW; ++e) acc = tfma(sc[e], y[r0 + e], acc);
    }
    const T d = group_sum(grp, acc);
    const T top = group_row<R>(grp, y, 0);
    const T tau = h0.g * tfma(-h0.beta, top, d);
#pragma unroll
    for (int r0 = 0; r0 < R; r0 += VW) {
        T tt[2], sc[2];
        src.get(r0, tt, sc);
#pragma unroll
        for (int e = 0; e < VW; ++e) {
            const T v = (r0 + e < VW && L::row_of(r0 + e, lane) == 0) ? h0.u : sc[e];
            y[r0 + e] = tfma(tau, v, y[r0 + e]);
        }
    }
    store_rows<T, R, G::W>(s_col, 64 * R * G::W, lane, true, y);
    return tfma(tau, h0.u, top);
}

template <typename T, int N, int Q, int R, int W, int PADM>
__device__ __noinline__ void slot_fill(VP_LDS SlotRec<T, N, Q> *rec, VP_LDS T *s_col, VP_LDS const T *s_t,
                                       VP_LDS const SlotConsts<T> *k, VP_LDS unsigned char *xch, const int prob,
                                       const T h0_beta, const T h0_u, const T h0_g) {
    using G = Grp<W>;
    G grp = G::make((unsigned char *)xch);
    const int lane = grp.gl;
    if constexpr (W > 1) __syncthreads();
    if (prob < 0) {
        if (lane == 0) {
            rec->prob = -1;
            rec->term = VP_TERM_NOT_RUN;
        }
        if constexpr (W > 1) __syncthreads();
        return;
    }
    using Src = RowSource<T, R, true, 0, 1, W, true, PADM>;
    Src src;
    src.t = (const T *)s_t;
    src.w = nullptr;
    src.m = k->m;
    src.lane = lane;
    src.vec = true;
    ConstReflector<T> h0;
    h0.beta = h0_beta;
    h0.u = h0_u;
    h0.g = h0_g;
    h0.live = true;
    const T qty0 = fill_slot_column<T, R, Src, G>(k->yw + (int64_t)prob * k->m, k->m, (T *)s_col, src, h0, grp);
    if (lane == 0) {
        const T *a0 = k->alpha + (int64_t)prob * Q;
#pragma unroll
        for (int i = 0; i < Q; ++i) {
            const T v = a0[i];
            rec->xt[i] = v;
            rec->x[i] = v;
            rec->diag[i] = T(1);
            rec->qtf[i] = T(0);
            rec->acnorm[i] = T(0);
            rec->ipvt[i] = i;
#pragma unroll
            for (int j = 0; j < Q; ++j) rec->Rj[i][j] = T(0);
        }
#pragma unroll
        for (int i = 0; i < N; ++i) {
            rec->cbest[i] = T(0);
            rec->cnew[i] = T(0);
        }
        rec->fnorm = rec->delta = rec->par = rec->xnorm = rec->gnorm = rec->pnorm = rec->prered = rec->dirder = T(0);
        rec->objective = T(0) / T(0);
        rec->fnorm1 = rec->actred = rec->ratio = T(0);
        rec->qty0 = qty0;
        if constexpr (VP_FIT2_PRE != 0) {
            const T pd = k->pre_delta;
#pragma unroll
            for (int i = 0; i < Q; ++i) {
                const T rti = frcp(a0[i]);
                rec->pre[2 * i] = rti;
                rec->pre[2 * i + 1] = texp(-div_refined(pd, a0[i], rti));
            }
            rec->pre[2 * Q] = rec->pre[2 * Q + 1] = T(0);
        }
        rec->flags = 1 | 2 | 4;
        rec->nfev = 0;
        rec->term = VP_TERM_NOT_RUN;
        rec->status = VP_ST_NOT_EVALUATED;
        rec->prob = prob;
        rec->trow = 0;
    }
    if constexpr (W > 1) __syncthreads();
}

template <typename T, int N, int Q, int GS, typename TO = T, bool GRAM = false>
__device__ __forceinline__ void slot_scalar_phase_inl(VP_LDS SlotRec<T, N, Q> *recs, VP_LDS const SlotConsts<T, TO> *k, const bool act = true) {
    const int lane = lane_id();
#ifdef VP_FIT2_CLOCKS
    long long sc0_ = __builtin_amdgcn_s_memtime();
    const bool sck_on_ = blockIdx.x == 0 && (threadIdx.x >> 6) == 0;
#define VP_SCK(i)                                                                                                      \
    do {                                                                                                               \
        const long long c1_ = __builtin_amdgcn_s_memtime();                                                           \
        if (sck_on_ && lane == 0) const_cast<SlotConsts<T, TO> *>((const SlotConsts<T, TO> *)k)->sck[i] += c1_ - sc0_;   \
        sc0_ = c1_;                                                                                                    \
    } while (0)
// ... 183 lines not shown
            delta = (!bad && first_tr && pnorm < delta) ? pnorm : delta;
            first_tr = bad ? first_tr : false;
#pragma unroll
            for (int i = 0; i < Q; ++i) xt[i] = bad ? xt[i] : x[i] - step[i];
        }
    }

    VP_SCK(4);
#pragma unroll
    for (int i = 0; i < Q; ++i) {
        s->x[i] = x[i];
        s->xt[i] = xt[i];
        s->diag[i] = diag[i];
    }
    if (accept_c) {
#pragma unroll
        for (int i = 0; i < N; ++i) s->cbest[i] = s->cnew[i];
    }
    if constexpr (!GRAM && VP_FIT2_PRE != 0) {
        const T pd = k->pre_delta;
#pragma unroll
        for (int i = 0; i < Q; ++i) {
            const T rti = frcp(xt[i]);
            s->pre[2 * i] = rti;
            s->pre[2 * i + 1] = texp(-div_refined(pd, xt[i], rti));
        }
        s->pre[2 * Q] = frcp(fnorm);
        s->pre[2 * Q + 1] = frcp(prered);
    }
    s->fnorm = fnorm;
    s->delta = delta;
    s->par = par;
    s->xnorm = xnorm;
    s->gnorm = gnorm;
    s->pnorm = pnorm;
    s->prered = prered;
    s->dirder = dirder;
    s->objective = objective;
    s->flags = (first ? 1 : 0) | (first_tr ? 2 : 0) | (first_update ? 4 : 0);
    s->nfev = nfev;
    s->term = term;
    s->status = status;
    s->trow = trow;

    if (term != 0) {
        vp_report rep;
        rep.termination = term;
        rep.n_evals = nfev;
        rep.objective = (double)objective;
        k->report[prob] = rep;
        double *cost_out = k->cost_out;
        int32_t *status_out = k->status;
        TO *alpha_out = k->alpha, *C_out = k->C_out;
        if (cost_out) cost_out[prob] = (double)objective;
        if (status_out && !VP_FITG_TIMELINE) status_out[prob] = status;
        int32_t *rescue = k->rescue;
        const int pslot = (s->pend[0] < 0) ? 0 : ((s->pend[1] < 0) ? 1 : -1);
        if (flagged && k->self_rescue != 0 && pslot >= 0) {
            s->pend[pslot] = (int)prob;
        } else if (flagged && k->self_rescue == 0 && rescue) {
            rescue_push(rescue, k->rescue_slot, prob);
        } else {
#pragma unroll
            for (int i = 0; i < Q; ++i) alpha_out[prob * Q + i] = (TO)x[i];
        }
        if (C_out) {
#pragma unroll
            for (int i = 0; i < N; ++i) C_out[prob * N + i] = (TO)s->cbest[i];
        }
    }
    VP_SCK(5);
}

template <typename T, int N, int Q, int GS, typename TO = T, bool GRAM = false>
__device__ __noinline__ void slot_scalar_phase(VP_LDS SlotRec<T, N, Q> *recs, VP_LDS const SlotConsts<T, TO> *k, const bool act = true) {
    slot_scalar_phase_inl<T, N, Q, GS, TO, GRAM>(recs, k, act);
}

#ifndef VP_LONE_TAIL_LINKAGE
#define VP_LONE_TAIL_LINKAGE __forceinline__
#endif
template <typename T, class M, int R, int PADM>
__device__ VP_LONE_TAIL_LINKAGE void fit2_lone_tail(VP_LDS SlotRec<T, M::N, M::Q> *rec, VP_LDS const T *s_col, VP_LDS const T *s_t,
                                            VP_LDS const SlotConsts<T> *kc, const M mdl, const T eps, const int uniform,
                                            const T h0_beta, const T h0_u, const T h0_g) {
    constexpr int N = M::N, P = M::P, Q = M::Q;
    constexpr int NC = N + P, YC = N - 1, DC = YC + 1;
    using G = Grp<1>;
    G grp = G::make(nullptr);
    const int lane = grp.gl;
    using Src = RowSource<T, R, true, 0, 1, 1, true, PADM>;
    Src src;
    src.t = (const T *)s_t;
    src.w = nullptr;
    src.m = kc->m;
    src.lane = lane;
    src.vec = true;
    src.set_uniform(uniform != 0);
    ConstReflector<T> h0;
    h0.beta = h0_beta;
    h0.u = h0_u;
    h0.g = h0_g;
    h0.live = true;
    const T ftol = kc->ftol, xtol = kc->xtol, gtol = kc->gtol, stepbound = kc->stepbound;
    const int scale_diag = uni(kc->scale_diag), max_fev = uni(kc->max_fev), mres = uni(kc->m);
    const int64_t prob = uni(rec->prob);
    const T qty0 = rec->qty0;
    T x[Q], xt[Q], diag[Q], qtf[Q], step[Q], acnorm[Q], cbest[N];
    T Rj[Q][Q];
    int ipvt[Q];
#pragma unroll
    for (int k = 0; k < Q; ++k) {
        xt[k] = rec->xt[k];
        step[k] = T(0);
    }
    T fnorm, delta, par, xnorm, gnorm, pnorm, prered, dirder, objective;
    bool first, first_tr, first_update;
    int nfev, term = VP_TERM_NOT_RUN, st_best = uni(rec->status), trow = uni(rec->trow);
    bool flagged = false;
    auto trace_row = [&](const T(&xx)[Q], T fn, T ratio) {
        double *trace = kc->trace;
        const int trace_rows = kc->trace_rows;
        if (trace && trow < trace_rows && lane == 0) {
            double *tr = trace + ((size_t)prob * trace_rows + trow) * (Q + 4);
#pragma unroll
            for (int k = 0; k < Q; ++k) tr[k] = (double)xx[k];
            tr[Q] = (double)fn;
            tr[Q + 1] = (double)ratio;
            tr[Q + 2] = (double)delta;
// ... 199 lines not shown
                }
                xnorm = enorm_small<T, Q>(tmpv);
                if (uni(!is_finite(xnorm))) {
                    term = VP_TERM_NUMERICAL;
                    break;
                }
                delta = (xnorm == T(0)) ? stepbound : stepbound * xnorm;
                first_update = false;
            } else if (scale_diag) {
#pragma unroll
                for (int k = 0; k < Q; ++k) diag[k] = tmax(diag[k], acnorm[k]);
            }
        }
        par = lmpar_any<T, Q>(Rj, ipvt, diag, qtf, delta, par, step, pnorm);
        if (uni(!is_finite(pnorm))) {
            term = VP_TERM_NUMERICAL;
            break;
        }
        {
            T wa[Q];
#pragma unroll
            for (int i = 0; i < Q; ++i) wa[i] = T(0);
#pragma unroll
            for (int j = 0; j < Q; ++j) {
                const T pj = dyn_get<Q>(step, ipvt[j]);
#pragma unroll
                for (int i = 0; i <= j; ++i) wa[i] = tfma(Rj[i][j], pj, wa[i]);
            }
            const T ifn = frcp(fnorm);
            const T t1 = enorm_small<T, Q>(wa) * ifn;
            const T temp1 = t1 * t1;
            const T t2 = (usqrt(par) * pnorm) * ifn;
            const T temp2 = t2 * t2;
            if (uni(!is_finite(temp1) || !is_finite(temp2))) {
                term = VP_TERM_NUMERICAL;
                break;
            }
            prered = temp1 + temp2 * T(2);
            dirder = -(temp1 + temp2);
        }
        if (first_tr && pnorm < delta) delta = pnorm;
        first_tr = false;
#pragma unroll
        for (int k = 0; k < Q; ++k) xt[k] = x[k] - step[k];
        park();
        asm volatile("s_waitcnt lgkmcnt(0)" ::: "memory");
    }
    if (lane == 0) {
        vp_report rep;
        rep.termination = term;
        rep.n_evals = nfev;
        rep.objective = (double)objective;
        kc->report[prob] = rep;
        double *cost_out = kc->cost_out;
        int32_t *status_out = kc->status;
        T *alpha_out = kc->alpha, *C_out = kc->C_out;
        if (cost_out) cost_out[prob] = (double)objective;
        if (status_out) status_out[prob] = st_best;
        const int pslot = (rec->pend[0] < 0) ? 0 : ((rec->pend[1] < 0) ? 1 : -1);
        if (flagged && kc->self_rescue != 0 && pslot >= 0) {
            rec->pend[pslot] = (int)prob;
        } else if (flagged && kc->self_rescue == 0 && kc->rescue) {
            rescue_push(kc->rescue, kc->rescue_slot, prob);
        } else {
#pragma unroll
            for (int k = 0; k < Q; ++k) alpha_out[prob * Q + k] = x[k];
        }
        if (C_out) {
#pragma unroll
            for (int k = 0; k < N; ++k) C_out[prob * N + k] = cbest[k];
        }
        rec->term = term;
    }
}

#ifndef VP_SELF_RESCUE
#define VP_SELF_RESCUE 1
#endif
template <typename T, class M, int W> inline constexpr bool fit2_self_rescue_v = VP_SELF_RESCUE && W == 1 && fit_rescue_v<T, M>;

template <typename T, class M, int R>
__device__ __noinline__ void fit2_refit_flagged(const FitArgs<T, M> *a, const int64_t b, T *s_t, T *s_y, LmState<T, M::N, M::Q> *st) {
    (void)fit_problem<T, M, R, 1, false, 0, true, false>(*a, b, s_t, s_y, nullptr, nullptr, st, false);
}

template <typename T, class M, int R, int W, int PADM, int GS, int NG, int WPS>
__global__ void __launch_bounds__(64 * W * NG, (WPS * W * NG) / 4 > 0 ? (WPS * W * NG) / 4 : 1) fit2_kernel(const Fit2Args<T, M> args) {
    static_assert(M::kConstLast && M::kDiagonalPairs, "slot kernel: multi-exponential + offset models");
    static_assert(W == 1 || NG == 1, "multi-wave groups synchronise with workgroup barriers: one group per workgroup");
    constexpr int N = M::N, P = M::P, Q = M::Q;
    constexpr int NC = N + P;
    constexpr int YC = N - 1;
    constexpr int DC = YC + 1;
    constexpr int MP = 64 * R * W;
    using Rec = SlotRec<T, N, Q>;
    extern __shared__ __attribute__((aligned(16))) unsigned char smem_raw[];
    T *s_t = reinterpret_cast<T *>(smem_raw);
    const int gi = (W == 1) ? (int)(threadIdx.x >> 6) : 0;
    T *s_y = s_t + MP + (size_t)gi * GS * MP;
    Rec *recs_all = reinterpret_cast<Rec *>(s_t + MP + (size_t)NG * GS * MP);
    Rec *recs = recs_all + (size_t)gi * GS;
    SlotConsts<T> *kc = reinterpret_cast<SlotConsts<T> *>(recs_all + (size_t)NG * GS);
    int *s_pop = reinterpret_cast<int *>(kc + 1);
    unsigned char *s_xch = reinterpret_cast<unsigned char *>(s_pop + ((GS + 3) / 4) * 4);
    using G = Grp<W>;
    G grp = G::make(s_xch);
    const int lane = grp.gl;
    const int gw = (int)blockIdx.x * NG + gi;
    auto group_sync = [&]() __attribute__((always_inline)) {
        if constexpr (W > 1) {
            __syncthreads();
        } else {
            __builtin_amdgcn_wave_barrier();
            asm volatile("s_waitcnt lgkmcnt(0)" ::: "memory");
        }
    };
    T eps_;
    int m_, uniform_;
    int64_t B_;
    {
        const FitArgs<T, M> &a = args.f;
        m_ = a.m;
        eps_ = a.eps;
        uniform_ = a.grid_uniform;
        B_ = a.B;
        T tmp[R];
        load_rows<T, R, W>(a.t, m_, lane, vec_aligned<T>(a.t, m_), tmp);
        store_rows<T, R, W>(s_t, MP, lane, true, tmp);
        if (threadIdx.x == 0) {
            kc->ftol = a.ftol;
            kc->xtol = a.xtol;
            kc->gtol = a.gtol;
            kc->stepbound = a.stepbound;
            kc->alpha = a.alpha;
            kc->rescue = a.rescue;
            kc->rescue_slot = a.rescue_slot;
            kc->self_rescue = (fit2_self_rescue_v<T, M, W> && a.rescue != nullptr) ? 1 : 0;
            kc->C_out = a.C_out;
            kc->cost_out = a.cost_out;
            kc->status = a.status;
            kc->report = a.report;
            kc->trace = a.trace;
            kc->yw = a.yw;
            kc->queue = args.queue;
            kc->B = a.B;
            kc->trace_rows = a.trace_rows;
            kc->scale_diag = a.scale_diag;
            kc->max_fev = a.patience * (Q + 1);
            kc->m = a.m;
#ifdef VP_FIT2_CLOCKS
            for (int i = 0; i < 6; ++i) kc->sck[i] = 0;
#endif
        }
    }
    __syncthreads();
    const int m = m_;
    using Src = RowSource<T, R, true, 0, 1, W, true, PADM>;
    Src src;
    src.t = s_t;
    src.w = nullptr;
    src.m = m;
    src.lane = lane;
    src.vec = true;
    src.set_uniform(uniform_ != 0);
    const ConstReflector<T> h0 = make_const_reflector<T, R, Src, G>(src, grp);
    const M mdl = args.f.mdl;
    if (threadIdx.x == 0) kc->pre_delta = src.uniform ? src.delta : T(0);
    __syncthreads();

    auto fill = [&](int s, int prob) __attribute__((always_inline)) {
        slot_fill<T, N, Q, R, W, PADM>((VP_LDS Rec *)(recs + s), (VP_LDS T *)(s_y + (size_t)s * MP), (VP_LDS const T *)s_t,
                                       (VP_LDS const SlotConsts<T> *)kc, (VP_LDS unsigned char *)s_xch, prob, h0.beta, h0.u,
                                       h0.g);
        if constexpr (W > 1) grp.phase = 0;
    };

    if (lane == 0) {
#pragma nounroll
        for (int s = 0; s < GS; ++s) recs[s].pend[0] = recs[s].pend[1] = -1;
    }
    int nactive = 0;
    bool queue_dry = false;
#pragma nounroll
    for (int s = 0; s < GS; ++s) {
        const int64_t prob = (int64_t)gw * GS + s;
        const bool have = prob < B_ && h0.live;
        fill(s, have ? (int)prob : -1);
// ... 36 lines not shown
            const T fnorm1 = usqrt(u.fn2);
            T actred = T(0), ratio = T(0);
            bool good = false;
            if (!first) {
                const T q1 = fnorm1 * (kPre ? rec->pre[2 * Q] : frcp(fnorm));
                actred = (fnorm1 * T(0.1) < fnorm) ? T(1) - q1 * q1 : T(-1);
                ratio = (prered == T(0)) ? T(0) : actred * (kPre ? rec->pre[2 * Q + 1] : frcp(prered));
                good = uni(ratio >= T(1.0e-4));
            }
            const bool need_jac = u.ok && (first || good);
            T Rj[Q][Q], acnorm[Q], qtf[Q];
            int ipvt[Q];
            if (need_jac) {
                residual_qcoords<T, R, N>(C[YC], u.e, grp);
                T zs[Q];
#pragma unroll
                for (int k = 0; k < Q; ++k) zs[k] = -u.c[k];
                jac_qrfac_scaled<T, R, Q, N>(reinterpret_cast<T(&)[Q][R]>(C[DC]), C[YC], zs, Rj, acnorm, ipvt, qtf, grp);
            }
            if (lane == 0) {
                rec->fnorm1 = fnorm1;
                rec->actred = actred;
                rec->ratio = ratio;
#pragma unroll
                for (int k = 0; k < N; ++k) rec->cnew[k] = u.c[k];
                int fl = fl_in & 7;
                if (u.ok) fl |= 8;
                if (need_jac) {
                    fl |= 16;
#pragma unroll
                    for (int k = 0; k < Q; ++k) {
                        rec->acnorm[k] = acnorm[k];
                        rec->qtf[k] = qtf[k];
                        rec->ipvt[k] = ipvt[k];
#pragma unroll
                        for (int j = 0; j < Q; ++j) rec->Rj[k][j] = Rj[k][j];
                    }
                }
                if (good) fl |= 32;
                rec->flags = fl;
            }
        }
        group_sync();
        VP_CK2(0);

        if (grp.wave == 0) slot_scalar_phase<T, N, Q, GS>((VP_LDS Rec *)recs, (VP_LDS const SlotConsts<T> *)kc);
        group_sync();
        VP_CK2(1);

        if constexpr (W > 1) {
            if (lane == 0) {
                for (int s = 0; s < GS; ++s)
                    s_pop[s] = (recs[s].prob >= 0 && recs[s].term != 0)
                                   ? __hip_atomic_fetch_add(kc->queue, 1, __ATOMIC_RELAXED, __HIP_MEMORY_SCOPE_AGENT)
                                   : -1;
            }
            __syncthreads();
        }
#pragma nounroll
        for (int s = 0; s < GS; ++s) {
            if (uni(recs[s].prob) < 0 || uni(recs[s].term) == 0) continue;
            int next = 0;
            if constexpr (W > 1) {
                next = uni(s_pop[s]);
            } else {
                if (lane == 0) next = __hip_atomic_fetch_add(kc->queue, 1, __ATOMIC_RELAXED, __HIP_MEMORY_SCOPE_AGENT);
                next = uni(next);
            }
            const bool have = (int64_t)next < B_;
            fill(s, have ? next : -1);
            if (!have) {
                nactive -= 1;
                queue_dry = true;
            }
        }
        group_sync();
        VP_CK2(2);
#ifndef VP_NO_LONE_TAIL
        if constexpr (W == 1) {
            if (queue_dry && nactive == 1) break;
        }
#endif
    }
#ifndef VP_NO_LONE_TAIL
    if constexpr (W == 1) {
        if (nactive == 1) {
#pragma nounroll
            for (int s = 0; s < GS; ++s) {
                if (uni(recs[s].prob) < 0) continue;
                fit2_lone_tail<T, M, R, PADM>((VP_LDS Rec *)(recs + s), (VP_LDS const T *)(s_y + (size_t)s * MP),
                                              (VP_LDS const T *)s_t, (VP_LDS const SlotConsts<T> *)kc, mdl, eps_, uniform_,
                                              h0.beta, h0.u, h0.g);
            }
        }
    }
#endif
    if constexpr (fit2_self_rescue_v<T, M, W>) {
        group_sync();
        int pend[2 * GS];
#pragma unroll
        for (int s = 0; s < GS; ++s) {
            pend[2 * s] = uni(recs[s].pend[0]);
            pend[2 * s + 1] = uni(recs[s].pend[1]);
        }
        group_sync();
        static_assert(sizeof(LmState<T, N, Q>) <= sizeof(Rec) * GS, "the parked LM state of the re-fit lives in the group's records");
#pragma nounroll
        for (int i = 0; i < 2 * GS; ++i) {
            const int pb_ = dyn_get<2 * GS>(pend, i);
            if (pb_ < 0) continue;
            fit2_refit_flagged<T, M, R>(&args.f, (int64_t)pb_, s_t, s_y, reinterpret_cast<LmState<T, N, Q> *>(recs));
        }
    }
#ifdef VP_FIT2_CLOCKS
    if (args.f.trace && blockIdx.x == 0 && threadIdx.x == 0) {
        double *tr = args.f.trace + (size_t)(args.f.trace_rows - 1) * (Q + 4);
        for (int i = 0; i < 3; ++i) tr[i] = (double)ck[i];
        double *tr2 = args.f.trace + (size_t)(args.f.trace_rows - 2) * (Q + 4);
        for (int i = 0; i < 6 && i < Q + 4; ++i) tr2[i] = (double)kc->sck[i];
    }
#endif
}

template <typename T, class M, int R, int W = 1> int launch_fit2(const LaunchParams &p) {
    if constexpr (!(M::kConstLast && M::kDiagonalPairs)) {
        return launch_fit<T, M, R, W>(p);
    } else {
        constexpr int NG = (W == 1) ? 4 : 1;
        constexpr int WPS = waves_for<T, R, M::N + M::P>();
        constexpr int BPC = (4 * WPS) / (W * NG) > 0 ? (4 * WPS) / (W * NG) : 1;
        constexpr int GS = fit2_slots<T, R, W, NG, BPC, (int)sizeof(SlotRec<T, M::N, M::Q>)>();
        const int64_t cap_groups = (int64_t)p.num_cus * BPC * NG;
        const bool small = (W == 1) ? (p.B <= 16 * cap_groups) : false;
        if (p.w || p.t_stride != 0 || !p.queue || p.fit_group == 1 || (p.fit_group != 2 && small))
            return launch_fit<T, M, R, W>(p);
        Fit2Args<T, M> args;
        FitArgs<T, M> &a = args.f;
        if (!bind_model(*p.model, a.mdl)) return VP_ERR_UNSUPPORTED;
        a.t = (const T *)p.t;
        a.w = nullptr;
        a.yw = (const T *)p.yw;
        a.alpha = (T *)p.alpha_out;
        a.C_out = (T *)p.C_out;
        a.cost_out = p.cost_out;
        a.status = p.status;
        a.report = p.report;
        a.m = p.m;
        a.B = p.B;
        a.t_stride = 0;
        a.w_stride = 0;
        a.eps = (T)p.eps;
        a.ftol = (T)p.opts->ftol;
        a.xtol = (T)p.opts->xtol;
        a.gtol = (T)p.opts->gtol;
        a.stepbound = (T)p.opts->stepbound;
        a.patience = p.opts->patience;
        a.scale_diag = p.opts->scale_diag;
        a.trace = p.trace;
        a.trace_rows = p.trace_rows;
        a.grid_uniform = p.grid_uniform;
        a.rescue = p.rescue;
        a.rescue_slot = p.rescue_slot;
        if (a.B <= 0) return VP_ERR_OK;
        if (p.rescue_used && !fit2_self_rescue_v<T, M, W>) *p.rescue_used = 1;
        const int64_t cap_blocks = (int64_t)p.num_cus * BPC;
        const int64_t need_blocks = (a.B + (int64_t)GS * NG - 1) / ((int64_t)GS * NG);
        const int64_t blocks = need_blocks < cap_blocks ? need_blocks : cap_blocks;
        args.queue = p.queue;
        args.waves_total = (int)(blocks * NG * W);
        if (hipMemsetD32Async((hipDeviceptr_t)p.queue, (int)(blocks * NG * GS), 1, p.stream) != hipSuccess) return VP_ERR_HIP;
        const size_t lds = (size_t)64 * R * W * sizeof(T) * (1 + (size_t)NG * GS) + (size_t)NG * GS * sizeof(SlotRec<T, M::N, M::Q>) +
                           sizeof(SlotConsts<T>) + (size_t)((GS + 3) / 4) * 4 * sizeof(int) + (size_t)group_xch_bytes<W>() + 16;
        if (lds > (size_t)(160 * 1024) / BPC) return launch_fit<T, M, R, W>(p);
#define VP_F2(PADM_)                                                                                                   \
    hipLaunchKernelGGL((fit2_kernel<T, M, R, W, PADM_, GS, NG, WPS>), dim3((unsigned)blocks), dim3(64 * W * NG), lds,   \
                       p.stream, args)
        if (p.m == 64 * R * W) VP_F2(1);
        else if (R > 2 && p.m > 64 * (R - 2) * W) VP_F2(2);
        else VP_F2(0);
#undef VP_F2
        return hipGetLastError() == hipSuccess ? VP_ERR_OK : VP_ERR_HIP;
    }
}

}
```

varpro_amd/csrc/vp_fitg.hpp:

```cpp
#pragma once
#include "vp_fit2.hpp"
#include "vp_lm_core.hpp"

#ifndef VP_FITG_IDLE_PARTNER
#define VP_FITG_IDLE_PARTNER 0
#endif
#ifndef VP_FITG_SCALAR_WAVES
#define VP_FITG_SCALAR_WAVES 1
#endif
#ifndef VP_FITG_CHOL_LMPAR
#define VP_FITG_CHOL_LMPAR 1
#endif
#ifndef VP_FITG_RESOLUTION_GUARD
#define VP_FITG_RESOLUTION_GUARD 1
#endif
#ifndef VP_FITG_PIVOT_NOISE
#define VP_FITG_PIVOT_NOISE 1.0e-10
#endif
#ifndef VP_FITG_RESOLUTION
#define VP_FITG_RESOLUTION 1.6e-11
#endif
#ifndef VP_FITG_CLOSED
#define VP_FITG_CLOSED 1
#endif
// ... 650 lines not shown
#ifndef VP_FITG_NS
#define VP_FITG_NS 32
#endif
#ifndef VP_FITG2_NWAVES
#define VP_FITG2_NWAVES 8
#endif
#ifndef VP_FITG_PARTS
#define VP_FITG_PARTS 4
#endif
#ifndef VP_FITG_SPLIT_AFTER
#define VP_FITG_SPLIT_AFTER 24
#endif
#ifndef VP_FITG_TIMELINE
#define VP_FITG_TIMELINE 0
#endif
#ifndef VP_FITG_OLD_FIRST
#define VP_FITG_OLD_FIRST 1
#endif
#ifndef VP_FITG_TAIL_LIVE
#define VP_FITG_TAIL_LIVE 7
#endif
constexpr int VP_FITG2_WAVES = VP_FITG2_NWAVES;

template <class M, int NS, bool UNIFORM, bool WEIGHTED>
__global__ void __launch_bounds__(64 * VP_FITG2_WAVES, VP_FITG2_WAVES == 8 ? 2 : 1) fitg2_kernel(const FitgArgs a) {
    constexpr int N = M::N, Q = M::Q, NE = M::N - 1;
    static_assert(M::kStatic && M::kConstLast && M::kDiagonalPairs && M::Q == NE, "exponentials + offset");
    static_assert(NS <= 64, "one lane of the scalar wave per slot");
    using GI = GramIdx<NE>;
    using Rec = SlotRec<double, N, Q>;
    using KC = SlotConsts<double, float>;
    __shared__ __attribute__((aligned(16))) double s_gram[NS][GI::NV];
    __shared__ __attribute__((aligned(16))) Rec s_recs[NS];
    __shared__ __attribute__((aligned(16))) KC s_kc;
    __shared__ double s_grid[NS][2];
    __shared__ double s_ymom[NS][2];
    __shared__ int s_state[NS];
    __shared__ int s_live;
    __shared__ __attribute__((aligned(16))) double s_pgram[NS][VP_FITG_PARTS][GI::NV];
    __shared__ int s_next[NS], s_done[NS];
    const int lane = lane_id();
    const int wv = (int)(threadIdx.x >> 6);
    const int m = a.m;
    VP_LDS Rec *recs = (VP_LDS Rec *)&s_recs[0];
    VP_LDS double *gram = (VP_LDS double *)&s_gram[0][0];
    VP_LDS const KC *kc = (VP_LDS const KC *)&s_kc;
    if (threadIdx.x == 0) {
        KC *k = &s_kc;
        k->ftol = a.ftol;
        k->xtol = a.xtol;
        k->gtol = a.gtol;
        k->stepbound = a.stepbound;
        k->alpha = a.alpha;
        k->C_out = a.C_out;
        k->cost_out = a.cost_out;
        k->status = a.status;
        k->report = a.report;
        k->trace = VP_FITG_TIMELINE ? nullptr : a.trace;
        k->yw = a.yw;
        k->queue = a.queue;
        k->rescue = nullptr;
        k->rescue_slot = 0;
        k->B = a.B;
        k->trace_rows = a.trace_rows;
        k->scale_diag = a.scale_diag;
        k->max_fev = a.patience * (Q + 1);
        k->m = a.m;
        k->eps = a.eps;
        s_live = 0;
    }
    __syncthreads();
    auto grid_of = [&](const int s, const int prob) __attribute__((always_inline)) {
        if constexpr (UNIFORM) {
            const float *tp = a.t + (int64_t)prob * a.t_stride;
            const double t0 = (double)tp[0];
            s_grid[s][0] = t0;
            s_grid[s][1] = ((double)tp[m - 1] - t0) / (double)(m - 1);
        }
    };
    if (wv == 0 && lane < NS) {
        const int64_t prob = (int64_t)blockIdx.x * a.gs_used + lane;
        const bool have = lane < a.gs_used && prob < a.B;
        if (have) {
            slotg_fill_lane<N, Q>(recs + lane, kc, (int)prob);
            grid_of(lane, (int)prob);
            __hip_atomic_fetch_add(&s_live, 1, __ATOMIC_RELAXED, __HIP_MEMORY_SCOPE_WORKGROUP);
        } else {
            s_recs[lane].prob = -1;
            s_recs[lane].term = VP_TERM_NOT_RUN;
        }
        s_state[lane] = have ? 1 : 0;
        s_next[lane] = VP_FITG_PARTS;
        s_done[lane] = 0;
    }
    __syncthreads();
    const int nchunk = (m + 255) / 256;
    const bool vec = (m & 3) == 0 && ((reinterpret_cast<uintptr_t>(a.yw) | reinterpret_cast<uintptr_t>(a.t) |
                                       reinterpret_cast<uintptr_t>(a.w)) & 15) == 0;
    auto lds_release = [&]() __attribute__((always_inline)) { asm volatile("s_waitcnt lgkmcnt(0)" ::: "memory"); };

    constexpr int NSC = VP_FITG_SCALAR_WAVES, GSW = NS / NSC;
    static_assert(NS % NSC == 0 && NSC < VP_FITG2_WAVES, "the pool divides evenly over the scalar waves");
    auto slot_advance = [&](const int slot, const bool on) __attribute__((always_inline)) {
        if (on) {
            int next_state = 1;
            if (s_recs[slot].term != 0) {
// ... 151 lines not shown
                asm volatile("" ::: "memory");
            }
            const int prob = uni(s_recs[s].prob);
            int ready_slot = -1;
            if (part < 0) {
                gram_pass<NE, UNIFORM, WEIGHTED>(a, recs + s, (VP_LDS const double *)&s_grid[s][0], gram + (size_t)s * GI::NV, prob, lane, m,
                                                 0, nchunk, vec, true, (VP_LDS double *)&s_ymom[s][0]);
                lds_release();
                ready_slot = s;
            } else {
                const int c0 = (int)((long)part * nchunk / VP_FITG_PARTS), c1 = (int)((long)(part + 1) * nchunk / VP_FITG_PARTS);
                gram_pass<NE, UNIFORM, WEIGHTED>(a, recs + s, (VP_LDS const double *)&s_grid[s][0],
                                                 (VP_LDS double *)&s_pgram[s][part][0], prob, lane, m, c0, c1, vec, part == 0,
                                                 (VP_LDS double *)&s_ymom[s][0]);
                lds_release();
                int d = 0;
                if (lane == 0) d = __hip_atomic_fetch_add(&s_done[s], 1, __ATOMIC_RELAXED, __HIP_MEMORY_SCOPE_WORKGROUP);
                if (uni(d) == VP_FITG_PARTS - 1) {
                    asm volatile("" ::: "memory");
                    for (int v = lane; v < GI::NV; v += 64) {
                        double t = s_pgram[s][0][v];
#pragma unroll
                        for (int q2 = 1; q2 < VP_FITG_PARTS; ++q2) t += s_pgram[s][q2][v];
                        s_gram[s][v] = t;
                    }
                    lds_release();
                    ready_slot = s;
                }
            }
            if (ready_slot >= 0) moments_ready(ready_slot);
            start = s + 1 >= NS ? 0 : s + 1;
#if VP_FITG_TIMELINE
            tl_busy += wall_clock64() - tl_a;
            if (part < 0) tl_pass += 1; else tl_parts += 1;
#endif
        }
        VP_TL_END();
    }
}

template <class M> int launch_fitg(const LaunchParams &p, double *dbg = nullptr) {
    if (p.S != 1 || !p.queue) return VP_ERR_UNSUPPORTED;
    FitgArgs a;
    a.t = (const float *)p.t;
    a.w = (const float *)p.w;
    a.yw = (const float *)p.yw;
    a.alpha = (float *)p.alpha_out;
    a.C_out = (float *)p.C_out;
    a.cost_out = p.cost_out;
    a.status = p.status;
    a.report = p.report;
    a.trace = p.trace;
    a.dbg = dbg;
    a.queue = p.queue;
    a.B = p.B;
    a.t_stride = p.t_stride;
    a.w_stride = p.w_stride;
    a.m = p.m;
    a.trace_rows = p.trace_rows;
    a.scale_diag = p.opts->scale_diag;
    a.patience = p.opts->patience;
    a.eps = p.eps;
    a.ftol = p.opts->ftol;
    a.xtol = p.opts->xtol;
    a.gtol = p.opts->gtol;
    a.stepbound = p.opts->stepbound;
    if (a.B <= 0) return VP_ERR_OK;
    const bool uniform = p.grid_uniform != 0 && p.m >= 3;
    const bool weighted = p.w != nullptr || (p.m & 3) != 0;
    constexpr int NS = VP_FITG_NS;
    const int64_t cap_groups = (int64_t)p.num_cus;
    int64_t ns_used = (a.B + cap_groups - 1) / cap_groups;
    if (ns_used > NS) ns_used = NS;
    if (ns_used < 1) ns_used = 1;
    a.gs_used = (int)ns_used;
    int64_t blocks = (a.B + ns_used - 1) / ns_used;
    if (blocks > cap_groups) blocks = cap_groups;
    if (hipMemsetD32Async((hipDeviceptr_t)p.queue, (int)(blocks * ns_used), 1, p.stream) != hipSuccess) return VP_ERR_HIP;
    const dim3 grid((unsigned)blocks), block(64 * VP_FITG2_WAVES);
    if (uniform && !weighted) hipLaunchKernelGGL((fitg2_kernel<M, NS, true, false>), grid, block, 0, p.stream, a);
    else if (uniform) hipLaunchKernelGGL((fitg2_kernel<M, NS, true, true>), grid, block, 0, p.stream, a);
    else if (!weighted) hipLaunchKernelGGL((fitg2_kernel<M, NS, false, false>), grid, block, 0, p.stream, a);
    else hipLaunchKernelGGL((fitg2_kernel<M, NS, false, true>), grid, block, 0, p.stream, a);
    return hipGetLastError() == hipSuccess ? VP_ERR_OK : VP_ERR_HIP;
}

}
```

varpro_amd/csrc/vp_generic.hpp:

```cpp
#pragma once
#include <cstring>

#include <mutex>

#include "vp_lm_core.hpp"

namespace vp {
namespace gen {

constexpr int TB = 256;
constexpr int MAXC = VP_MAX_BASIS + 1 + VP_MAX_PAIRS + VP_MAX_PARAMS;
constexpr int MAXV = VP_MAX_BASIS + 1 + VP_MAX_PAIRS;

template <typename T> struct GenArgs {
    vp_model_desc mdl;
    int P;
    int pb[VP_MAX_PAIRS], pa[VP_MAX_PAIRS], pp[VP_MAX_PAIRS];
    const T *t, *w, *yw;
    int S;
    const T *alpha;
    T *alpha_io;
    T *r_out, *J_out, *C_out;
    const T *C_in;
    double *cost_out;
    int32_t *status;
    vp_report *report;
    T *Phi_out, *dPhi_out;
    int skip_invariant, n_phi_cols;
    T *ws;
    int64_t ws_cols;
    int m;
    int64_t B;
    int64_t t_stride, w_stride;
    T eps;
    LmOpts<T> lm;
    double *trace;
    int trace_rows;
    int phase;
    void *lm_state;
    double *acc;
    int32_t *nactive;
    int64_t S_global;
    int ext;
    const T *ext_phi, *ext_dphi;
    int ext_rows;
    const int32_t *list;
    int list_slot;
    int list_first;
    int scale_cols;
    int ws_lds;
};
#ifndef VP_GEN_LDS_KB
#define VP_GEN_LDS_KB 150
#endif
constexpr size_t kGenLdsMax = (size_t)VP_GEN_LDS_KB * 1024;
template <typename T> __device__ __forceinline__ T *gen_workspace(const GenArgs<T> &a, unsigned char *dyn_lds) {
    return a.ws_lds ? reinterpret_cast<T *>(dyn_lds) : a.ws + (int64_t)blockIdx.x * a.ws_cols * a.m;
}
__host__ __device__ constexpr int gen_nacc(int q) { return 2 + q * q + q; }

template <typename T> __device__ __forceinline__ T g_exp(T x);
template <> __device__ __forceinline__ double g_exp(double x) { return texp(x); }
template <> __device__ __forceinline__ float g_exp(float x) { return texp(x); }

template <typename T>
__device__ __forceinline__ void basis_eval(int kind, T t, T p0, T p1, T &f, T &d0, T &d1) {
    d0 = T(0);
    d1 = T(0);
    switch (kind) {
    case VP_BASIS_CONST: f = T(1); break;
    case VP_BASIS_EXP_DECAY: {
        const T rt = frcp(p0);
        f = g_exp(-div_refined(t, p0, rt));
        d0 = (f * t) * (rt * rt);
    } break;
    case VP_BASIS_EXP_RATE:
        f = g_exp(-p0 * t);
        d0 = -t * f;
        break;
    case VP_BASIS_EXP_COS: {
        const T ex = g_exp(-p0 * t);
        T sn_, cs_;
        tsincos(p1 * t, sn_, cs_);
        f = ex * cs_;
        d0 = f * (-t);
        d1 = -t * ex * sn_;
    } break;
    default: {
        const T ph = p0 * t + p1;
        T cs;
        tsincos(ph, f, cs);
        d0 = t * cs;
        d1 = cs;
    } break;
    }
}

template <typename T> struct GenShared {
    T part[MAXV][TB / 64];
    unsigned long long mx[VP_MAX_BASIS];
    T sw[VP_MAX_BASIS][VP_MAX_BASIS], sv[VP_MAX_BASIS][VP_MAX_BASIS];
    T red[MAXV];
    T f[MAXV];
// ... 520 lines not shown
        if (q == 0) {
            if (tid == 0) s_term = VP_TERM_NO_PARAMETERS;
            __syncthreads();
        }
        while (s_term == 0) {
            evaluate<T>(a, sh, ws, b, true);
            if (tid == 0) {
                const T fnorm1 = tsqrt(sh.fn2);
                bool need = false;
                VP_GEN_DISPATCH(q, {
                    need = lm_after_eval<T, VP_MAX_BASIS, QQ, false>(S, a.lm, fnorm1, sh.ok != 0, (long)m);
                    if (S.accepted)
                        for (int k = 0; k < n; ++k) cbest[k] = sh.c[k];
                    if (a.trace && s_trow < a.trace_rows) {
                        double *tr = a.trace + ((size_t)b * a.trace_rows + s_trow) * (q + 4);
                        for (int k = 0; k < QQ; ++k) tr[k] = (double)S.xt[k];
                        tr[q] = (double)fnorm1;
                        tr[q + 1] = 0.0 / 0.0;
                        tr[q + 2] = (double)S.delta;
                        tr[q + 3] = (double)S.par;
                    }
                    ++s_trow;
                    s_term = S.term;
                });
                s_need_jac = need ? 1 : 0;
            }
            __syncthreads();
            if (s_term != 0) break;
            if (s_need_jac) jac_qrfac<T>(a, sh, ws);
            if (tid == 0) {
                VP_GEN_DISPATCH(q, {
                    if (s_need_jac) {
                        for (int k = 0; k < QQ; ++k) {
                            S.acnorm[k] = sh.acnorm[k];
                            S.qtf[k] = sh.qtf[k];
                            S.ipvt[k] = sh.ipvt[k];
                            for (int l = 0; l < QQ; ++l) S.Rj[k][l] = sh.Rj[k][l];
                        }
                    }
                    lm_next_step<T, VP_MAX_BASIS, QQ, false>(S, a.lm, s_need_jac != 0);
                    s_term = S.term;
                    for (int k = 0; k < QQ; ++k) sh.alpha[k] = S.xt[k];
                });
            }
            __syncthreads();
        }
        if (tid == 0) {
            vp_report rep;
            VP_GEN_DISPATCH(q, {
                rep.termination = S.term;
                rep.n_evals = S.nfev;
                rep.objective = (double)S.objective;
                for (int k = 0; k < QQ; ++k) a.alpha_io[b * q + k] = S.x[k];
                if (a.status) a.status[b] = S.status;
            });
            if (q == 0) {
                rep.termination = VP_TERM_NO_PARAMETERS;
                rep.n_evals = 0;
                rep.objective = 0.0 / 0.0;
                if (a.status) a.status[b] = VP_ST_NOT_EVALUATED;
            }
            a.report[b] = rep;
            if (a.cost_out) a.cost_out[b] = rep.objective;
            if (a.C_out)
                for (int k = 0; k < n; ++k) a.C_out[b * n + k] = cbest[k];
        }
        __syncthreads();
    }
}

template <typename T> __global__ void __launch_bounds__(TB) gen_mrhs_fit_kernel(const GenArgs<T> a) {
    __shared__ GenShared<T> sh;
    __shared__ LmAny<T> lm;
    __shared__ int s_term, s_trow, s_okall;
    __shared__ double s_acc[2 + VP_MAX_PARAMS * VP_MAX_PARAMS + VP_MAX_PARAMS];
    const int tid = (int)threadIdx.x, m = a.m, n = a.mdl.n_basis, q = a.mdl.n_params, P = a.P, NS = a.S;
    const int NCQ = n + 1 + P;
    const int phase = a.phase;
    const long mres = (long)m * (long)(a.S_global > 0 ? a.S_global : NS);
    extern __shared__ __attribute__((aligned(16))) unsigned char gen_dyn_lds[];
    T *ws = gen_workspace<T>(a, gen_dyn_lds);
    auto col = [&](int c) { return ws + (int64_t)c * m; };
    LmAny<T> *gstate = reinterpret_cast<LmAny<T> *>(a.lm_state);
    for (int64_t b = blockIdx.x; b < a.B; b += gridDim.x) {
        if (tid == 0) {
            if (phase <= 1) {
                T a0[VP_MAX_PARAMS];
                for (int k = 0; k < q; ++k) a0[k] = a.alpha_io[b * q + k];
                VP_GEN_DISPATCH(q, (lm_init<T, VP_MAX_BASIS, QQ>(S, a0)));
                for (int k = 0; k < q; ++k) sh.alpha[k] = a0[k];
                s_term = (q == 0) ? VP_TERM_NO_PARAMETERS : 0;
                if (phase == 1) {
                    gstate[b] = lm;
                    if (q > 0) atomicAdd(a.nactive, 1);
                }
            } else {
                lm = gstate[b];
                s_term = 0;
                VP_GEN_DISPATCH(q, {
                    s_term = S.term;
                    for (int k = 0; k < QQ; ++k) sh.alpha[k] = (phase == 4) ? S.x[k] : S.xt[k];
                });
                if (q == 0) s_term = VP_TERM_NO_PARAMETERS;
            }
            s_trow = 0;
        }
        __syncthreads();
        if (phase == 1) continue;
        while (s_term == 0 && phase != 4) {
            if (phase != 3) {
                if (tid == 0) {
                    for (int i = 0; i < gen_nacc(q); ++i) s_acc[i] = 0.0;
                    s_okall = 1;
                }
                __syncthreads();
                for (int s = 0; s < NS; ++s) {
                    evaluate<T>(a, sh, ws, b, false, b * NS + s);
                    for (int k = 0; k < q; ++k) {
// ... 297 lines not shown
            s_ok = ok ? 1 : 0;
            sh.fn2 = chi2;
        }
        __syncthreads();
        if (sa.sigma_out) {
            build(false);
            const T s0 = s_ok ? tsqrt(sh.fn2) : T(0) / T(0);
            for (int i = tid; i < m; i += TB) {
                T acc = T(0);
                for (int c = 0; c < K; ++c) {
                    T v = T(0);
                    for (int r = 0; r <= c; ++r) v = tfma(Ri[r][c], col(r)[i], v);
                    acc = tfma(v, v, acc);
                }
                sa.sigma_out[b * (int64_t)m + i] = s0 * tsqrt(acc);
            }
        }
        __syncthreads();
    }
}

template <typename T> inline bool fill_args(const LaunchParams &p, GenArgs<T> &a) {
    std::memset(&a, 0, sizeof(a));
    a.mdl = *p.model;
    int np = 0;
    if (p.ext) {
        if (p.ext_np > VP_MAX_PAIRS || !p.ext_phi) return false;
        for (; np < p.ext_np; ++np) {
            a.pb[np] = p.ext_pb[np];
            a.pa[np] = 0;
            a.pp[np] = p.ext_pp[np];
        }
        a.ext = 1;
        a.ext_phi = (const T *)p.ext_phi;
        a.ext_dphi = (const T *)p.ext_dphi;
        a.ext_rows = p.ext_rows > 0 ? p.ext_rows : p.m;
    } else
    for (int j = 0; j < p.model->n_basis; ++j)
        for (int k = 0; k < VP_MAX_BASIS_PARAMS; ++k)
            if (p.model->param[j][k] >= 0) {
                if (np >= VP_MAX_PAIRS) return false;
                a.pb[np] = j;
                a.pa[np] = k;
                a.pp[np] = p.model->param[j][k];
                ++np;
            }
    a.P = np;
    a.t = (const T *)p.t;
    a.w = (const T *)p.w;
    a.yw = (const T *)p.yw;
    a.S = p.S > 0 ? p.S : 1;
    a.alpha = (const T *)p.alpha;
    a.alpha_io = (T *)p.alpha_out;
    a.r_out = (T *)p.r_out;
    a.J_out = (T *)p.J_out;
    a.C_out = (T *)p.C_out;
    a.cost_out = p.cost_out;
    a.status = p.status;
    a.report = p.report;
    a.Phi_out = (T *)p.Phi_out;
    a.dPhi_out = (T *)p.dPhi_out;
    a.ws = (T *)p.gen_ws;
    a.ws_cols = p.model->n_basis + 1 + np + p.model->n_params;
    a.m = p.m;
    a.B = p.B;
    a.t_stride = p.t_stride;
    a.w_stride = p.w_stride;
    a.eps = (T)p.eps;
    if (p.opts) {
        a.lm.ftol = (T)p.opts->ftol;
        a.lm.xtol = (T)p.opts->xtol;
        a.lm.gtol = (T)p.opts->gtol;
        a.lm.stepbound = (T)p.opts->stepbound;
        a.lm.patience = p.opts->patience;
        a.lm.scale_diag = p.opts->scale_diag;
    }
    a.trace = p.trace;
    a.trace_rows = p.trace_rows;
    a.list = p.gen_list;
    a.list_slot = p.gen_list_slot;
    a.list_first = p.gen_list_first;
    a.scale_cols = p.gen_scale_cols;
    return true;
}

template <typename T, class K> inline size_t gen_lds_for(GenArgs<T> &a, K kernel) {
    const size_t need = (size_t)a.ws_cols * (size_t)a.m * sizeof(T);
    a.ws_lds = 0;
    if (need == 0 || need > kGenLdsMax) return 0;
    static const void *seen[16];
    static bool seen_ok[16];
    static int nseen = 0;
    static std::mutex mtx;
    std::lock_guard<std::mutex> lock(mtx);
    bool attr_ok = false, found = false;
    for (int i = 0; i < nseen; ++i)
        if (seen[i] == (const void *)kernel) {
            attr_ok = seen_ok[i];
            found = true;
        }
    if (!found) {
        attr_ok = hipFuncSetAttribute((const void *)kernel, hipFuncAttributeMaxDynamicSharedMemorySize, (int)kGenLdsMax) == hipSuccess;
        if (!attr_ok) (void)hipGetLastError();
        if (nseen < 16) {
            seen[nseen] = (const void *)kernel;
            seen_ok[nseen] = attr_ok;
// ... 81 lines not shown
```

varpro_amd/csrc/vp_kernels.hpp:

```cpp
#pragma once
#include <initializer_list>

#include "vp_core.hpp"

namespace vp {

#ifndef VP_TWO_WAVE_VGPRS
#define VP_TWO_WAVE_VGPRS 200
#endif
template <typename T, int R, int NC> constexpr int waves_for() {
    return (NC * R * (int)(sizeof(T) / 4) <= VP_TWO_WAVE_VGPRS) ? 2 : 1;
}
#ifndef VP_RT_ONE_WAVE
#define VP_RT_ONE_WAVE 1
#endif
template <typename T, class M, int R, int NC> constexpr int model_waves_for() {
    return (VP_RT_ONE_WAVE && !M::kStatic && R >= 12) ? 1 : waves_for<T, R, NC>();
}
template <typename T, int R, int NC, int W> constexpr int group_waves_per_eu() {
    return W >= 4 ? ((waves_for<T, R, NC>() * W) / 4 > 0 ? (waves_for<T, R, NC>() * W) / 4 : 1) : waves_for<T, R, NC>();
}

struct LaunchParams {
    const vp_model_desc *model;
    const void *t;
    const void *w;
    const void *yw;
    const void *alpha;
    void *alpha_out;
    void *r_out;
    void *J_out;
    void *C_out;
    double *cost_out;
    int32_t *status;
    void *Phi_out;
    void *dPhi_out;
    vp_report *report;
    const vp_lm_opts *opts;
    double *trace;
    int trace_rows;
    int fit_group;
    int *queue;
    double *gram_dbg;
    int num_cus;
    void *gen_ws;
    int gen_phase;
    void *gen_lm_state;
    double *gen_acc;
    int32_t *gen_nactive;
    int gen_blocks;
    const void *mrhs_ws;
    const void *mrhs_fws;
    const void *mrhs_io;
    int32_t *mrhs_hflag;
    int mrhs_mode;
    int mrhs_init;
    int mrhs_gx;
    int64_t mrhs_S_global;
    int basis_flags;
    int m;
    int S;
    int64_t B;
    int64_t t_stride;
    int64_t w_stride;
    double eps;
    int grid_uniform;
    const void *ext_phi;
    const void *ext_dphi;
    const int32_t *ext_pb;
    const int32_t *ext_pp;
    int ext;
    int ext_np;
    int ext_rows;
    int32_t *rescue;
    int rescue_slot;
    int *rescue_used;
    const int32_t *gen_list;
    int gen_list_slot;
    int gen_list_first;
    int gen_scale_cols;
    hipStream_t stream;
};
// ... 599 lines not shown
```

Before: 31.58 million fits/s.

## Fit kernel reads user alpha and writes results directly into user buffers

Adds vp_fit_into, which lets the fit kernel read the initial guess from the caller's buffer and write alpha, coefficients and reports straight into the caller's device arrays. This removes the device-to-device copies before and after the fit and the Python-side clone of alpha. The per-launch queue memset is replaced by a static queue base plus a self-resetting counter. The summary kernel is changed to use last-block reduction instead of a memset plus atomics. In exchange it adds state that must stay consistent across launches, such as resetting the queue counter and the fit_direct mode, and any error there could corrupt work distribution.

```diff
diff --git a/bindings/rust/varpro_hip.rs b/bindings/rust/varpro_hip.rs
--- a/bindings/rust/varpro_hip.rs
+++ b/bindings/rust/varpro_hip.rs
@@ -63,6 +63,8 @@
     pub fn vp_lm_opts_default(o: *mut vp_lm_opts, dtype: i32);
     pub fn vp_fit(h: *mut vp_batch, opts: *const vp_lm_opts, alpha_inout: *mut c_void, c_out: *mut c_void,
         rep: *mut vp_report) -> i32;
+    pub fn vp_fit_into(h: *mut vp_batch, opts: *const vp_lm_opts, alpha0: *const c_void, alpha_out: *mut c_void,
+        c_out: *mut c_void, rep: *mut vp_report) -> i32;
     pub fn vp_best_fit(h: *mut vp_batch, fit_out: *mut c_void) -> i32;
     pub fn vp_debug_gram_evaluate(h: *mut vp_batch, alpha: *const c_void, out: *mut f64) -> i32;
     pub fn vp_summary(h: *mut vp_batch, out: *mut f64) -> i32;
diff --git a/include/varpro_hip.h b/include/varpro_hip.h
--- a/include/varpro_hip.h
+++ b/include/varpro_hip.h
@@ -146,6 +146,7 @@
 int vp_fit_active_set(vp_batch *h, int32_t *index_out, int32_t *count_out);
 
 int vp_fit(vp_batch *h, const vp_lm_opts *opts, void *alpha_inout, void *C_out, vp_report *rep);
+int vp_fit_into(vp_batch *h, const vp_lm_opts *opts, const void *alpha0, void *alpha_out, void *C_out, vp_report *rep);
 
 int vp_fit_trace(vp_batch *h, const vp_lm_opts *opts, void *alpha_inout, void *C_out, vp_report *rep,
                  double *trace_out, int trace_rows);
diff --git a/varpro_amd/_lib.py b/varpro_amd/_lib.py
--- a/varpro_amd/_lib.py
+++ b/varpro_amd/_lib.py
@@ -34,7 +34,7 @@
 
 ABI_SYMBOLS = [
     "vp_batch_create", "vp_batch_destroy", "vp_set_params", "vp_params", "vp_residuals", "vp_jacobian",
-    "vp_linear_coeffs", "vp_weighted_data", "vp_set_observations", "vp_cost", "vp_evaluate", "vp_basis", "vp_lm_opts_default", "vp_fit", "vp_fit_trace",
+    "vp_linear_coeffs", "vp_weighted_data", "vp_set_observations", "vp_cost", "vp_evaluate", "vp_basis", "vp_lm_opts_default", "vp_fit", "vp_fit_into", "vp_fit_trace",
     "vp_best_fit", "vp_statistics", "vp_summary", "vp_summary_device", "vp_global_fit_condition", "vp_set_rhs_allreduce", "vp_set_fit_kernel", "vp_set_timing", "vp_last_kernel_ms", "vp_synchronize", "vp_last_error",
     "vp_last_error_detail", "vp_version", "vp_device_count",
     "vp_batch_create_external", "vp_set_params_with_basis", "vp_jacobian_with_derivatives", "vp_evaluate_with_basis",
@@ -122,6 +122,7 @@
     lib.vp_lm_opts_default.argtypes = [C.POINTER(LmOpts), C.c_int]
     lib.vp_lm_opts_default.restype = None
     lib.vp_fit.argtypes = [vp, C.POINTER(LmOpts), vp, vp, vp]
+    lib.vp_fit_into.argtypes = [vp, C.POINTER(LmOpts), vp, vp, vp, vp]
     lib.vp_fit_trace.argtypes = [vp, C.POINTER(LmOpts), vp, vp, vp, vp, C.c_int]
     lib.vp_best_fit.argtypes = [vp, vp]
     lib.vp_debug_gram_evaluate.argtypes = [vp, vp, vp]
diff --git a/varpro_amd/batch.py b/varpro_amd/batch.py
--- a/varpro_amd/batch.py
+++ b/varpro_amd/batch.py
@@ -350,17 +350,19 @@
         solver = solver or LevenbergMarquardt(self.np_dtype)
         opts = solver._c()
         a = self._as_array(alpha0).reshape(self.B, self.q)
-        a = a.clone() if _is_torch(a) else a.copy()
         Cm = self._empty((self.B, self.S, self.n)) if want_coefficients else None
         if self.device_mode:
+            a0, a = a, torch.empty_like(a)
+            self._fit_guess = a0
             rep_t = torch.empty((self.B, 16), dtype=torch.uint8, device=self._torch_device())
-            check(self.lib.vp_fit(self._h, C.byref(opts), self._ptr(a), self._ptr(Cm), self._ptr(rep_t)))
+            check(self.lib.vp_fit_into(self._h, C.byref(opts), self._ptr(a0), self._ptr(a), self._ptr(Cm), self._ptr(rep_t)))
             self._have_params = True
             rep = rep_t
             if Cm is not None and self.single_rhs:
                 Cm = Cm.reshape(self.B, self.n)
             return a, Cm, rep
         else:
+            a = a.clone() if _is_torch(a) else a.copy()
             rep = np.zeros(self.B, dtype=REPORT_DTYPE)
             check(self.lib.vp_fit(self._h, C.byref(opts), self._ptr(a), self._ptr(Cm), C.c_void_p(rep.ctypes.data)))
             self._have_params = True
diff --git a/varpro_amd/cpp/varpro.hpp b/varpro_amd/cpp/varpro.hpp
--- a/varpro_amd/cpp/varpro.hpp
+++ b/varpro_amd/cpp/varpro.hpp
@@ -314,6 +314,13 @@
         check(vp_fit(h_, &solver.o, alpha_inout.data(), nullptr, rep.data()));
         return rep;
     }
+    std::vector<vp_report> fit_into(const std::vector<double> &alpha0, std::vector<double> &alpha_out,
+                                    const LevenbergMarquardt &solver = LevenbergMarquardt()) {
+        std::vector<vp_report> rep((size_t)B);
+        alpha_out.resize(alpha0.size());
+        check(vp_fit_into(h_, &solver.o, alpha0.data(), alpha_out.data(), nullptr, rep.data()));
+        return rep;
+    }
     struct Statistics {
         std::vector<double> covariance;
         std::vector<double> reduced_chi2;
diff --git a/varpro_amd/csrc/vp_api.hip b/varpro_amd/csrc/vp_api.hip
--- a/varpro_amd/csrc/vp_api.hip
+++ b/varpro_amd/csrc/vp_api.hip
@@ -94,7 +94,9 @@
     }
 }
 
-__global__ void summary_kernel(const vp_report *__restrict__ rep, int64_t B, double *__restrict__ out4) {
+constexpr int kSummaryBlocks = 1024;
+__global__ void summary_kernel(const vp_report *__restrict__ rep, int64_t B, double *__restrict__ out4, double *part,
+                               unsigned int *arrived) {
     double c = 0, ok = 0, bad = 0, ev = 0;
     for (int64_t b = blockIdx.x * (int64_t)blockDim.x + threadIdx.x; b < B; b += (int64_t)gridDim.x * blockDim.x) {
         const vp_report r = rep[b];
@@ -114,9 +116,23 @@
             for (int k = 0; k < 4; ++k) sh[k][threadIdx.x] += sh[k][threadIdx.x + off];
         __syncthreads();
     }
-    if (threadIdx.x == 0)
-        for (int k = 0; k < 4; ++k) atomicAdd(&out4[k], sh[k][0]);
-}
+    __shared__ bool last;
+    if (threadIdx.x == 0) {
+        for (int k = 0; k < 4; ++k) part[4 * blockIdx.x + k] = sh[k][0];
+        __threadfence();
+        last = atomicAdd(arrived, 1u) == gridDim.x - 1;
+    }
+    __syncthreads();
+    if (!last) return;
+    __threadfence();
+    if (threadIdx.x < 4) {
+        double tot = 0;
+        for (unsigned g = 0; g < gridDim.x; ++g) tot += __hip_atomic_load(&part[4 * g + threadIdx.x], __ATOMIC_RELAXED, __HIP_MEMORY_SCOPE_AGENT);
+        out4[threadIdx.x] = tot;
+    }
+    if (threadIdx.x == 0) *arrived = 0u;
+}
+constexpr size_t kSummaryDoubles = 4 + 4 * (size_t)kSummaryBlocks + 1;
 
 __global__ void mrhs_reduce_partials_kernel(const double *part, int gx, int nacc, int64_t B, double *tot) {
     const int64_t idx = blockIdx.x * (int64_t)blockDim.x + threadIdx.x;
@@ -183,6 +199,7 @@
     void *d_gen_lm;
     int32_t *d_gen_nactive;
     int fit_kernel;
+    int fit_direct;
     int *d_queue;
     int num_cus;
     void *tmp_a, *tmp_b;
@@ -495,8 +512,8 @@
     DeviceGuard dev_guard__;                                                                                          \
     if (int rc__ = dev_guard__.enter((h)->device)) return rc__
 
-int mrhs_fit(vp_batch *h, const vp_lm_opts *opts, void *alpha_inout, void *C_out, vp_report *rep, double *trace_out,
-             int trace_rows) {
+int mrhs_fit(vp_batch *h, const vp_lm_opts *opts, const void *alpha0, void *alpha_inout, void *C_out, vp_report *rep,
+             double *trace_out, int trace_rows) {
     if (!h->have_mrhs && !h->kern->mrhs_fit_whole) return fail(VP_ERR_UNSUPPORTED, "no MRHS kernels for this (model, m)");
     vp_lm_opts o;
     if (opts) o = *opts;
@@ -512,13 +529,13 @@
         std::memset(h->h_io, 0, sizeof(MrhsIo));
     }
     if (use_io) {
-        h->h_io->alpha_in = alpha_inout;
+        h->h_io->alpha_in = const_cast<void *>(alpha0);
         h->h_io->alpha_out = alpha_inout;
         h->h_io->C_out = C_out;
         h->h_io->rep_out = rep;
     } else {
         std::memset(h->h_io, 0, sizeof(MrhsIo));
-        VP_HIP(hipMemcpyAsync(h->d_alpha, alpha_inout, (size_t)h->B * h->q * ts, kin, h->stream));
+        VP_HIP(hipMemcpyAsync(h->d_alpha, alpha0, (size_t)h->B * h->q * ts, kin, h->stream));
     }
     LaunchParams p;
     fill_params(h, p);
@@ -1034,8 +1051,10 @@
         VP_TRY(hipMalloc((void **)&h->d_status, (size_t)B * sizeof(int32_t)));
     }
     VP_TRY(hipMalloc((void **)&h->d_report, (size_t)B * sizeof(vp_report)));
-    VP_TRY(hipMalloc((void **)&h->d_sum4, 4 * sizeof(double)));
-    VP_TRY(hipMalloc((void **)&h->d_queue, sizeof(int)));
+    VP_TRY(hipMalloc((void **)&h->d_sum4, kSummaryDoubles * sizeof(double)));
+    VP_TRY(hipMemsetAsync(h->d_sum4, 0, kSummaryDoubles * sizeof(double), h->stream));
+    VP_TRY(hipMalloc((void **)&h->d_queue, 4 * sizeof(int)));
+    VP_TRY(hipMemsetAsync(h->d_queue, 0, 4 * sizeof(int), h->stream));
     if (kern->uses_gen_ws && !ext) {
         if (int rc = ensure_gen_ws(h)) {
             vp_batch_destroy(h);
@@ -1540,8 +1559,13 @@
     return VP_ERR_OK;
 }
 
+static int fit_impl(vp_batch *h, const vp_lm_opts *opts, const void *alpha0, void *alpha_inout, void *C_out, vp_report *rep,
+                    double *trace_out, int trace_rows);
 int vp_fit(vp_batch *h, const vp_lm_opts *opts, void *alpha_inout, void *C_out, vp_report *rep) {
-    return vp_fit_trace(h, opts, alpha_inout, C_out, rep, nullptr, 0);
+    return fit_impl(h, opts, alpha_inout, alpha_inout, C_out, rep, nullptr, 0);
+}
+int vp_fit_into(vp_batch *h, const vp_lm_opts *opts, const void *alpha0, void *alpha_out, void *C_out, vp_report *rep) {
+    return fit_impl(h, opts, alpha0, alpha_out, C_out, rep, nullptr, 0);
 }
 
 namespace {
@@ -1583,12 +1607,17 @@
 
 int vp_fit_trace(vp_batch *h, const vp_lm_opts *opts, void *alpha_inout, void *C_out, vp_report *rep,
                  double *trace_out, int trace_rows) {
+    return fit_impl(h, opts, alpha_inout, alpha_inout, C_out, rep, trace_out, trace_rows);
+}
+
+static int fit_impl(vp_batch *h, const vp_lm_opts *opts, const void *alpha0, void *alpha_inout, void *C_out, vp_report *rep,
+                    double *trace_out, int trace_rows) {
     VP_ENTER(h);
     VP_NOT_EXTERNAL(h, "vp_fit");
-    if (!alpha_inout) return fail(VP_ERR_INVALID, "null alpha");
+    if (!alpha0 || !alpha_inout) return fail(VP_ERR_INVALID, "null alpha");
     if (h->m_user && (int64_t)h->q > h->m_user * h->S) {
         const size_t ts = tsize(h->dtype);
-        VP_HIP(hipMemcpyAsync(h->d_alpha, alpha_inout, (size_t)h->B * h->q * ts,
+        VP_HIP(hipMemcpyAsync(h->d_alpha, alpha0, (size_t)h->B * h->q * ts,
                               device_ptrs(h) ? hipMemcpyDeviceToDevice : hipMemcpyHostToDevice, h->stream));
         if (int rc = run_evaluate(h, nullptr, nullptr, h->d_C)) return rc;
         OutBuf trw;
@@ -1604,21 +1633,33 @@
         h->have_params = true;
         h->r_valid = false;
         h->have_report = true;
+        if (alpha_inout != alpha0)
+            if (int rc = copy_out(h, alpha_inout, h->d_alpha, (size_t)h->B * h->q * ts)) return rc;
         if (int rc = copy_out(h, C_out, h->d_C, (size_t)h->B * h->S * h->n * ts)) return rc;
         if (int rc = copy_out(h, rep, h->d_report, (size_t)h->B * sizeof(vp_report))) return rc;
         return trw.finish(h);
     }
-    if (h->S != 1) return mrhs_fit(h, opts, alpha_inout, C_out, rep, trace_out, trace_rows);
+    if (h->S != 1) return mrhs_fit(h, opts, alpha0, alpha_inout, C_out, rep, trace_out, trace_rows);
     if (!h->kern->fit && !h->kern->fit_single) return fail(VP_ERR_UNSUPPORTED, "no fit kernel for this model");
     vp_lm_opts o;
     if (opts) o = *opts;
     else vp_lm_opts_default(&o, h->dtype);
     const size_t ts = tsize(h->dtype);
-    VP_HIP(hipMemcpyAsync(h->d_alpha, alpha_inout, (size_t)h->B * h->q * ts,
-                          device_ptrs(h) ? hipMemcpyDeviceToDevice : hipMemcpyHostToDevice, h->stream));
+    const bool want_direct = device_ptrs(h) && !h->m_user && !(trace_out && trace_rows > 0);
+    if (!(want_direct && h->fit_direct == 1))
+        VP_HIP(hipMemcpyAsync(h->d_alpha, alpha0, (size_t)h->B * h->q * ts,
+                              device_ptrs(h) ? hipMemcpyDeviceToDevice : hipMemcpyHostToDevice, h->stream));
     LaunchParams p;
     fill_params(h, p);
     p.alpha_out = h->d_alpha;
+    int direct = 0;
+    if (want_direct) {
+        p.alpha_in = alpha0;
+        p.alpha_user = alpha_inout;
+        p.C_user = C_out;
+        p.report_user = rep;
+        p.io_direct = &direct;
+    }
     p.C_out = h->d_C;
     p.cost_out = h->d_cost_bs;
     p.status = h->d_status_bs;
@@ -1638,15 +1679,23 @@
     p.rescue_used = &list_used;
     Timer tm(h, VP_KERNEL_FIT);
     int rc = fit_fn(p);
+    if (want_direct) h->fit_direct = direct ? 1 : 2;
+    p.io_direct = nullptr;
+    if (!direct) p.alpha_in = p.alpha_user = p.C_user = p.report_user = nullptr;
     if (rc == VP_ERR_OK && list_used) rc = rescue_refit(h, p);
     tm.stop();
-    if (rc != VP_ERR_OK) return fail(rc, "fit kernel launch failed");
+    if (rc != VP_ERR_OK) {
+        (void)hipMemsetAsync(h->d_queue, 0, 2 * sizeof(int), h->stream);
+        return fail(rc, "fit kernel launch failed");
+    }
     h->have_params = true;
     h->r_valid = false;
     h->have_report = true;
-    if (int rc2 = copy_out(h, alpha_inout, h->d_alpha, (size_t)h->B * h->q * ts)) return rc2;
-    if (int rc2 = copy_out(h, C_out, h->d_C, (size_t)h->B * h->n * ts)) return rc2;
-    if (int rc2 = copy_out(h, rep, h->d_report, (size_t)h->B * sizeof(vp_report))) return rc2;
+    if (!direct) {
+        if (int rc2 = copy_out(h, alpha_inout, h->d_alpha, (size_t)h->B * h->q * ts)) return rc2;
+        if (int rc2 = copy_out(h, C_out, h->d_C, (size_t)h->B * h->n * ts)) return rc2;
+        if (int rc2 = copy_out(h, rep, h->d_report, (size_t)h->B * sizeof(vp_report))) return rc2;
+    }
     if (int rc2 = tr.finish(h)) return rc2;
     return VP_ERR_OK;
 }
@@ -1937,13 +1986,18 @@
     return VP_ERR_OK;
 }
 
+static int launch_summary(vp_batch *h, double *out4) {
+    const unsigned grid = (unsigned)std::max<int64_t>(1, std::min<int64_t>((h->B + 255) / 256, kSummaryBlocks));
+    hipLaunchKernelGGL(summary_kernel, dim3(grid), dim3(256), 0, h->stream, h->d_report, h->B, out4, h->d_sum4 + 4,
+                       reinterpret_cast<unsigned int *>(h->d_sum4 + 4 + 4 * (size_t)kSummaryBlocks));
+    VP_HIP(hipGetLastError());
+    return 0;
+}
+
 int vp_summary(vp_batch *h, double out[4]) {
     VP_ENTER(h);
     if (!h->have_report) return fail(VP_ERR_INVALID, "vp_summary requires a completed vp_fit");
-    VP_HIP(hipMemsetAsync(h->d_sum4, 0, 4 * sizeof(double), h->stream));
-    const unsigned grid = (unsigned)std::min<int64_t>((h->B + 255) / 256, 1024);
-    hipLaunchKernelGGL(summary_kernel, dim3(grid), dim3(256), 0, h->stream, h->d_report, h->B, h->d_sum4);
-    VP_HIP(hipGetLastError());
+    if (int rc = launch_summary(h, h->d_sum4)) return rc;
     VP_HIP(hipMemcpyAsync(out, h->d_sum4, 4 * sizeof(double), hipMemcpyDeviceToHost, h->stream));
     VP_HIP(hipStreamSynchronize(h->stream));
     return VP_ERR_OK;
@@ -1962,10 +2016,7 @@
     VP_ENTER(h);
     if (!h->have_report) return fail(VP_ERR_INVALID, "vp_summary_device requires a completed vp_fit");
     if (!dev_out4) return fail(VP_ERR_INVALID, "null output");
-    VP_HIP(hipMemsetAsync(dev_out4, 0, 4 * sizeof(double), h->stream));
-    const unsigned grid = (unsigned)std::min<int64_t>((h->B + 255) / 256, 1024);
-    hipLaunchKernelGGL(summary_kernel, dim3(grid), dim3(256), 0, h->stream, h->d_report, h->B, dev_out4);
-    VP_HIP(hipGetLastError());
+    if (int rc = launch_summary(h, dev_out4)) return rc;
     return VP_ERR_OK;
 }
 
@@ -1990,10 +2041,7 @@
     VP_ENTER(h);
     if (!out) return fail(VP_ERR_INVALID, "null output");
     if (!h->have_report) return fail(VP_ERR_INVALID, "vp_reduce_cost requires a completed vp_fit");
-    VP_HIP(hipMemsetAsync(h->d_sum4, 0, 4 * sizeof(double), h->stream));
-    const unsigned grid = (unsigned)std::min<int64_t>((h->B + 255) / 256, 1024);
-    hipLaunchKernelGGL(summary_kernel, dim3(grid), dim3(256), 0, h->stream, h->d_report, h->B, h->d_sum4);
-    VP_HIP(hipGetLastError());
+    if (int rc = launch_summary(h, h->d_sum4)) return rc;
     if (rccl_comm) {
         vp_nccl_allreduce_t ar = resolve_nccl_allreduce();
         if (!ar) return fail(VP_ERR_UNSUPPORTED, "ncclAllReduce not found: link librccl or make librccl.so.1 loadable");
@@ -2009,6 +2057,10 @@
     if (!h) return fail(VP_ERR_INVALID, "null handle");
     if (which != VP_FIT_KERNEL_AUTO && which != VP_FIT_KERNEL_WAVE && which != VP_FIT_KERNEL_SLOTS)
         return fail(VP_ERR_INVALID, "vp_set_fit_kernel: unknown kernel selector");
+    if (which != h->fit_kernel) {
+        VP_ENTER(h);
+        VP_HIP(hipMemsetAsync(h->d_queue, 0, 2 * sizeof(int), h->stream));
+    }
     h->fit_kernel = which;
     return VP_ERR_OK;
 }
diff --git a/varpro_amd/csrc/vp_fit.hpp b/varpro_amd/csrc/vp_fit.hpp
--- a/varpro_amd/csrc/vp_fit.hpp
+++ b/varpro_amd/csrc/vp_fit.hpp
@@ -931,6 +931,13 @@
     int rescue_slot;
 };
 
+template <typename T> struct FitIo {
+    const T *alpha_in;
+    T *alpha_user;
+    T *C_user;
+    vp_report *report_user;
+};
+
 template <typename T, int N, int Q> struct LmState {
     T x[Q], diag[Q], qtf[Q], acnorm[Q], cbest[N];
     T Rj[Q][Q];
@@ -943,7 +950,7 @@
 template <typename T, class M> inline constexpr bool fit_rescue_v = M::kStatic && M::kConstLast && M::kDiagonalPairs;
 
 template <typename T, class M, int R, int W, bool WEIGHTED, int PADM, bool RESCUE, bool SELF>
-__device__ __forceinline__ bool fit_problem(const FitArgs<T, M> &a, const int64_t b, T *s_t, T *s_y, T *s_w, unsigned char *xch,
+__device__ __forceinline__ bool fit_problem(const FitArgs<T, M> &a, const FitIo<T> &io, const int64_t b, T *s_t, T *s_y, T *s_w, unsigned char *xch,
                                             LmState<T, M::N, M::Q> *st, const bool stage_grid) {
     static_assert(!(WEIGHTED && PADM != 0), "PADM is a unit-weight specialisation");
     static_assert(!RESCUE || fit_rescue_v<T, M>, "the scaled re-fit needs the constant-first sweep and diagonal pairs");
@@ -996,7 +1003,7 @@
     int ipvt[Q];
 #pragma unroll
     for (int k = 0; k < Q; ++k) {
-        xt[k] = a.alpha[b * Q + k];
+        xt[k] = io.alpha_in[b * Q + k];
         x[k] = xt[k];
         diag[k] = T(1);
         qtf[k] = T(0);
@@ -1324,26 +1331,41 @@
         rep.n_evals = nfev;
         rep.objective = (double)objective;
         a.report[b] = rep;
+        if (io.report_user) io.report_user[b] = rep;
         if (a.cost_out) a.cost_out[b] = (double)objective;
         if (a.status) a.status[b] = st_best;
     }
     if (lane == 0) {
         if (flagged && (SELF || a.rescue != nullptr)) {
-            if (!SELF) rescue_push(a.rescue, a.rescue_slot, b);
+            if (!SELF) {
+                if (io.alpha_in != a.alpha) {
+#pragma unroll
+                    for (int k = 0; k < Q; ++k) a.alpha[b * Q + k] = io.alpha_in[b * Q + k];
+                }
+                rescue_push(a.rescue, a.rescue_slot, b);
+            }
         } else {
 #pragma unroll
             for (int k = 0; k < Q; ++k) a.alpha[b * Q + k] = x[k];
+            if (io.alpha_user) {
+#pragma unroll
+                for (int k = 0; k < Q; ++k) io.alpha_user[b * Q + k] = x[k];
+            }
         }
         if (a.C_out) {
 #pragma unroll
             for (int k = 0; k < N; ++k) a.C_out[b * N + a.mdl.out_index(k)] = cbest[k];
         }
+        if (io.C_user) {
+#pragma unroll
+            for (int k = 0; k < N; ++k) io.C_user[b * N + a.mdl.out_index(k)] = cbest[k];
+        }
     }
     return flagged;
 }
 
 template <typename T, class M, int R, int W, bool WEIGHTED, int PADM = 0, bool RESCUE = false>
-__global__ void __launch_bounds__(64 * W, (model_waves_for<T, M, R, M::N + 1 + M::P>())) fit_kernel(const FitArgs<T, M> a) {
+__global__ void __launch_bounds__(64 * W, (model_waves_for<T, M, R, M::N + 1 + M::P>())) fit_kernel(const FitArgs<T, M> a, const FitIo<T> io) {
     constexpr int MP = 64 * R * W;
     extern __shared__ __attribute__((aligned(16))) unsigned char smem_raw[];
     T *s_t = reinterpret_cast<T *>(smem_raw);
@@ -1359,12 +1381,21 @@
     } else {
         if (b >= a.B) return;
     }
-    (void)fit_problem<T, M, R, W, WEIGHTED, PADM, RESCUE, false>(a, b, s_t, s_y, s_w, s_after, st, true);
+    (void)fit_problem<T, M, R, W, WEIGHTED, PADM, RESCUE, false>(a, io, b, s_t, s_y, s_w, s_after, st, true);
 }
 
 template <typename T, class M, int R, int W> constexpr size_t fit_lds_bytes(bool weighted) {
     return (size_t)(weighted ? 3 : 2) * 64 * R * W * sizeof(T) + ((group_xch_bytes<W>() + 15) / 16) * 16 +
            (size_t)W * sizeof(LmState<T, M::N, M::Q>);
+}
+template <typename T> inline FitIo<T> bind_user_arrays(const LaunchParams &p) {
+    FitIo<T> io;
+    io.alpha_in = p.alpha_in ? (const T *)p.alpha_in : (const T *)p.alpha_out;
+    io.alpha_user = (T *)p.alpha_user;
+    io.C_user = (T *)p.C_user;
+    io.report_user = p.report_user;
+    if (p.io_direct) *p.io_direct = 1;
+    return io;
 }
 template <typename T, class M, int R, int W = 1> int launch_fit(const LaunchParams &p) {
     FitArgs<T, M> a;
@@ -1375,6 +1406,7 @@
     a.yw = (const T *)p.yw;
     a.alpha = (T *)p.alpha_out;
     a.C_out = (T *)p.C_out;
+    const FitIo<T> io = bind_user_arrays<T>(p);
     a.cost_out = p.cost_out;
     a.status = p.status;
     a.report = p.report;
@@ -1397,12 +1429,12 @@
     if (a.B <= 0) return VP_ERR_OK;
     if (p.rescue_used) *p.rescue_used = 1;
     const size_t lds = fit_lds_bytes<T, M, R, W>(p.w != nullptr);
-    if (p.w) hipLaunchKernelGGL((fit_kernel<T, M, R, W, true>), dim3((unsigned)a.B), dim3(64 * W), lds, p.stream, a);
+    if (p.w) hipLaunchKernelGGL((fit_kernel<T, M, R, W, true>), dim3((unsigned)a.B), dim3(64 * W), lds, p.stream, a, io);
     else if (p.m == 64 * R * W)
-        hipLaunchKernelGGL((fit_kernel<T, M, R, W, false, 1>), dim3((unsigned)a.B), dim3(64 * W), lds, p.stream, a);
+        hipLaunchKernelGGL((fit_kernel<T, M, R, W, false, 1>), dim3((unsigned)a.B), dim3(64 * W), lds, p.stream, a, io);
     else if (R > 2 && p.m > 64 * (R - 2) * W)
-        hipLaunchKernelGGL((fit_kernel<T, M, R, W, false, 2>), dim3((unsigned)a.B), dim3(64 * W), lds, p.stream, a);
-    else hipLaunchKernelGGL((fit_kernel<T, M, R, W, false>), dim3((unsigned)a.B), dim3(64 * W), lds, p.stream, a);
+        hipLaunchKernelGGL((fit_kernel<T, M, R, W, false, 2>), dim3((unsigned)a.B), dim3(64 * W), lds, p.stream, a, io);
+    else hipLaunchKernelGGL((fit_kernel<T, M, R, W, false>), dim3((unsigned)a.B), dim3(64 * W), lds, p.stream, a, io);
     return hipGetLastError() == hipSuccess ? VP_ERR_OK : VP_ERR_HIP;
 }
 
@@ -1418,6 +1450,7 @@
         a.yw = (const T *)p.yw;
         a.alpha = (T *)p.alpha_out;
         a.C_out = (T *)p.C_out;
+        const FitIo<T> io = bind_user_arrays<T>(p);
         a.cost_out = p.cost_out;
         a.status = p.status;
         a.report = p.report;
@@ -1438,7 +1471,7 @@
         a.rescue = p.rescue;
         a.rescue_slot = p.rescue_slot;
         const size_t lds = fit_lds_bytes<T, M, R, W>(false);
-        hipLaunchKernelGGL((fit_kernel<T, M, R, W, false, 0, true>), dim3(kFitRescueGrid), dim3(64 * W), lds, p.stream, a);
+        hipLaunchKernelGGL((fit_kernel<T, M, R, W, false, 0, true>), dim3(kFitRescueGrid), dim3(64 * W), lds, p.stream, a, io);
         return hipGetLastError() == hipSuccess ? VP_ERR_OK : VP_ERR_HIP;
     }
 }
diff --git a/varpro_amd/csrc/vp_fit2.hpp b/varpro_amd/csrc/vp_fit2.hpp
--- a/varpro_amd/csrc/vp_fit2.hpp
+++ b/varpro_amd/csrc/vp_fit2.hpp
@@ -39,7 +39,8 @@
 template <typename T, class M> struct Fit2Args {
     FitArgs<T, M> f;
     int *queue;
-    int waves_total;
+    int static_count;
+    int groups_total;
 };
 
 
@@ -47,6 +48,9 @@
     T ftol, xtol, gtol, stepbound;
     TO *alpha;
     TO *C_out;
+    FitIo<TO> io;
+    int queue_base;
+    int groups_total;
     double *cost_out;
     int32_t *status;
     vp_report *report;
@@ -128,7 +132,7 @@
     h0.live = true;
     const T qty0 = fill_slot_column<T, R, Src, G>(k->yw + (int64_t)prob * k->m, k->m, (T *)s_col, src, h0, grp);
     if (lane == 0) {
-        const T *a0 = k->alpha + (int64_t)prob * Q;
+        const T *a0 = k->io.alpha_in + (int64_t)prob * Q;
 #pragma unroll
         for (int i = 0; i < Q; ++i) {
             const T v = a0[i];
@@ -418,6 +422,9 @@
         double *cost_out = k->cost_out;
         int32_t *status_out = k->status;
         TO *alpha_out = k->alpha, *C_out = k->C_out;
+        TO *alpha_user = k->io.alpha_user, *C_user = k->io.C_user;
+        vp_report *report_user = k->io.report_user;
+        if (report_user) report_user[prob] = rep;
         if (cost_out) cost_out[prob] = (double)objective;
         if (status_out && !VP_FITG_TIMELINE) status_out[prob] = status;
         int32_t *rescue = k->rescue;
@@ -425,14 +432,27 @@
         if (flagged && k->self_rescue != 0 && pslot >= 0) {
             s->pend[pslot] = (int)prob;
         } else if (flagged && k->self_rescue == 0 && rescue) {
+            const TO *a0 = k->io.alpha_in;
+            if (a0 != alpha_out) {
+#pragma unroll
+                for (int i = 0; i < Q; ++i) alpha_out[prob * Q + i] = a0[prob * Q + i];
+            }
             rescue_push(rescue, k->rescue_slot, prob);
         } else {
 #pragma unroll
             for (int i = 0; i < Q; ++i) alpha_out[prob * Q + i] = (TO)x[i];
+            if (alpha_user) {
+#pragma unroll
+                for (int i = 0; i < Q; ++i) alpha_user[prob * Q + i] = (TO)x[i];
+            }
         }
         if (C_out) {
 #pragma unroll
             for (int i = 0; i < N; ++i) C_out[prob * N + i] = (TO)s->cbest[i];
+        }
+        if (C_user) {
+#pragma unroll
+            for (int i = 0; i < N; ++i) C_user[prob * N + i] = (TO)s->cbest[i];
         }
     }
     VP_SCK(5);
@@ -441,6 +461,14 @@
 template <typename T, int N, int Q, int GS, typename TO = T, bool GRAM = false>
 __device__ __noinline__ void slot_scalar_phase(VP_LDS SlotRec<T, N, Q> *recs, VP_LDS const SlotConsts<T, TO> *k, const bool act = true) {
     slot_scalar_phase_inl<T, N, Q, GS, TO, GRAM>(recs, k, act);
+}
+
+template <typename T> __device__ __noinline__ void slot_queue_leave(VP_LDS const SlotConsts<T> *k) {
+    int *q = k->queue;
+    if (__hip_atomic_fetch_add(q + 1, 1, __ATOMIC_RELAXED, __HIP_MEMORY_SCOPE_AGENT) == k->groups_total - 1) {
+        q[0] = 0;
+        q[1] = 0;
+    }
 }
 
 #ifndef VP_LONE_TAIL_LINKAGE
@@ -746,23 +774,39 @@
         rep.n_evals = nfev;
         rep.objective = (double)objective;
         kc->report[prob] = rep;
+        vp_report *report_user = kc->io.report_user;
+        if (report_user) report_user[prob] = rep;
         double *cost_out = kc->cost_out;
         int32_t *status_out = kc->status;
         T *alpha_out = kc->alpha, *C_out = kc->C_out;
+        T *alpha_user = kc->io.alpha_user, *C_user = kc->io.C_user;
         if (cost_out) cost_out[prob] = (double)objective;
         if (status_out) status_out[prob] = st_best;
         const int pslot = (rec->pend[0] < 0) ? 0 : ((rec->pend[1] < 0) ? 1 : -1);
         if (flagged && kc->self_rescue != 0 && pslot >= 0) {
             rec->pend[pslot] = (int)prob;
         } else if (flagged && kc->self_rescue == 0 && kc->rescue) {
+            const T *a0 = kc->io.alpha_in;
+            if (a0 != alpha_out) {
+#pragma unroll
+                for (int k = 0; k < Q; ++k) alpha_out[prob * Q + k] = a0[prob * Q + k];
+            }
             rescue_push(kc->rescue, kc->rescue_slot, prob);
         } else {
 #pragma unroll
             for (int k = 0; k < Q; ++k) alpha_out[prob * Q + k] = x[k];
+            if (alpha_user) {
+#pragma unroll
+                for (int k = 0; k < Q; ++k) alpha_user[prob * Q + k] = x[k];
+            }
         }
         if (C_out) {
 #pragma unroll
             for (int k = 0; k < N; ++k) C_out[prob * N + k] = cbest[k];
+        }
+        if (C_user) {
+#pragma unroll
+            for (int k = 0; k < N; ++k) C_user[prob * N + k] = cbest[k];
         }
         rec->term = term;
     }
@@ -774,12 +818,13 @@
 template <typename T, class M, int W> inline constexpr bool fit2_self_rescue_v = VP_SELF_RESCUE && W == 1 && fit_rescue_v<T, M>;
 
 template <typename T, class M, int R>
-__device__ __noinline__ void fit2_refit_flagged(const FitArgs<T, M> *a, const int64_t b, T *s_t, T *s_y, LmState<T, M::N, M::Q> *st) {
-    (void)fit_problem<T, M, R, 1, false, 0, true, false>(*a, b, s_t, s_y, nullptr, nullptr, st, false);
+__device__ __noinline__ void fit2_refit_flagged(const FitArgs<T, M> *a, const FitIo<T> *io, const int64_t b, T *s_t, T *s_y,
+                                                LmState<T, M::N, M::Q> *st) {
+    (void)fit_problem<T, M, R, 1, false, 0, true, false>(*a, *io, b, s_t, s_y, nullptr, nullptr, st, false);
 }
 
 template <typename T, class M, int R, int W, int PADM, int GS, int NG, int WPS>
-__global__ void __launch_bounds__(64 * W * NG, (WPS * W * NG) / 4 > 0 ? (WPS * W * NG) / 4 : 1) fit2_kernel(const Fit2Args<T, M> args) {
+__global__ void __launch_bounds__(64 * W * NG, (WPS * W * NG) / 4 > 0 ? (WPS * W * NG) / 4 : 1) fit2_kernel(const Fit2Args<T, M> args, const FitIo<T> io) {
     static_assert(M::kConstLast && M::kDiagonalPairs, "slot kernel: multi-exponential + offset models");
     static_assert(W == 1 || NG == 1, "multi-wave groups synchronise with workgroup barriers: one group per workgroup");
     constexpr int N = M::N, P = M::P, Q = M::Q;
@@ -827,6 +872,9 @@
             kc->gtol = a.gtol;
             kc->stepbound = a.stepbound;
             kc->alpha = a.alpha;
+            kc->io = io;
+            kc->queue_base = args.static_count;
+            kc->groups_total = args.groups_total;
             kc->rescue = a.rescue;
             kc->rescue_slot = a.rescue_slot;
             kc->self_rescue = (fit2_self_rescue_v<T, M, W> && a.rescue != nullptr) ? 1 : 0;
@@ -969,7 +1017,7 @@
             if (lane == 0) {
                 for (int s = 0; s < GS; ++s)
                     s_pop[s] = (recs[s].prob >= 0 && recs[s].term != 0)
-                                   ? __hip_atomic_fetch_add(kc->queue, 1, __ATOMIC_RELAXED, __HIP_MEMORY_SCOPE_AGENT)
+                                   ? kc->queue_base + __hip_atomic_fetch_add(kc->queue, 1, __ATOMIC_RELAXED, __HIP_MEMORY_SCOPE_AGENT)
                                    : -1;
             }
             __syncthreads();
@@ -981,7 +1029,7 @@
             if constexpr (W > 1) {
                 next = uni(s_pop[s]);
             } else {
-                if (lane == 0) next = __hip_atomic_fetch_add(kc->queue, 1, __ATOMIC_RELAXED, __HIP_MEMORY_SCOPE_AGENT);
+                if (lane == 0) next = kc->queue_base + __hip_atomic_fetch_add(kc->queue, 1, __ATOMIC_RELAXED, __HIP_MEMORY_SCOPE_AGENT);
                 next = uni(next);
             }
             const bool have = (int64_t)next < B_;
@@ -1026,9 +1074,11 @@
         for (int i = 0; i < 2 * GS; ++i) {
             const int pb_ = dyn_get<2 * GS>(pend, i);
             if (pb_ < 0) continue;
-            fit2_refit_flagged<T, M, R>(&args.f, (int64_t)pb_, s_t, s_y, reinterpret_cast<LmState<T, N, Q> *>(recs));
-        }
-    }
+            fit2_refit_flagged<T, M, R>(&args.f, &kc->io, (int64_t)pb_, s_t, s_y, reinterpret_cast<LmState<T, N, Q> *>(recs));
+        }
+    }
+    if constexpr (W > 1) __syncthreads();
+    if (lane == 0) slot_queue_leave<T>((VP_LDS const SlotConsts<T> *)kc);
 #ifdef VP_FIT2_CLOCKS
     if (args.f.trace && blockIdx.x == 0 && threadIdx.x == 0) {
         double *tr = args.f.trace + (size_t)(args.f.trace_rows - 1) * (Q + 4);
@@ -1079,19 +1129,20 @@
         a.rescue = p.rescue;
         a.rescue_slot = p.rescue_slot;
         if (a.B <= 0) return VP_ERR_OK;
+        const FitIo<T> io = bind_user_arrays<T>(p);
         if (p.rescue_used && !fit2_self_rescue_v<T, M, W>) *p.rescue_used = 1;
         const int64_t cap_blocks = (int64_t)p.num_cus * BPC;
         const int64_t need_blocks = (a.B + (int64_t)GS * NG - 1) / ((int64_t)GS * NG);
         const int64_t blocks = need_blocks < cap_blocks ? need_blocks : cap_blocks;
         args.queue = p.queue;
-        args.waves_total = (int)(blocks * NG * W);
-        if (hipMemsetD32Async((hipDeviceptr_t)p.queue, (int)(blocks * NG * GS), 1, p.stream) != hipSuccess) return VP_ERR_HIP;
+        args.static_count = (int)(blocks * NG * GS);
+        args.groups_total = (int)(blocks * NG);
         const size_t lds = (size_t)64 * R * W * sizeof(T) * (1 + (size_t)NG * GS) + (size_t)NG * GS * sizeof(SlotRec<T, M::N, M::Q>) +
                            sizeof(SlotConsts<T>) + (size_t)((GS + 3) / 4) * 4 * sizeof(int) + (size_t)group_xch_bytes<W>() + 16;
         if (lds > (size_t)(160 * 1024) / BPC) return launch_fit<T, M, R, W>(p);
 #define VP_F2(PADM_)                                                                                                   \
     hipLaunchKernelGGL((fit2_kernel<T, M, R, W, PADM_, GS, NG, WPS>), dim3((unsigned)blocks), dim3(64 * W * NG), lds,   \
-                       p.stream, args)
+                       p.stream, args, io)
         if (p.m == 64 * R * W) VP_F2(1);
         else if (R > 2 && p.m > 64 * (R - 2) * W) VP_F2(2);
         else VP_F2(0);
diff --git a/varpro_amd/csrc/vp_fitg.hpp b/varpro_amd/csrc/vp_fitg.hpp
--- a/varpro_amd/csrc/vp_fitg.hpp
+++ b/varpro_amd/csrc/vp_fitg.hpp
@@ -726,6 +726,11 @@
         k->gtol = a.gtol;
         k->stepbound = a.stepbound;
         k->alpha = a.alpha;
+        k->io.alpha_in = a.alpha;
+        k->io.alpha_user = nullptr;
+        k->io.C_user = nullptr;
+        k->io.report_user = nullptr;
+        k->queue_base = 0;
         k->C_out = a.C_out;
         k->cost_out = a.cost_out;
         k->status = a.status;
@@ -983,7 +988,7 @@
     a.report = p.report;
     a.trace = p.trace;
     a.dbg = dbg;
-    a.queue = p.queue;
+    a.queue = p.queue + 2;
     a.B = p.B;
     a.t_stride = p.t_stride;
     a.w_stride = p.w_stride;
@@ -1007,7 +1012,7 @@
     a.gs_used = (int)ns_used;
     int64_t blocks = (a.B + ns_used - 1) / ns_used;
     if (blocks > cap_groups) blocks = cap_groups;
-    if (hipMemsetD32Async((hipDeviceptr_t)p.queue, (int)(blocks * ns_used), 1, p.stream) != hipSuccess) return VP_ERR_HIP;
+    if (hipMemsetD32Async((hipDeviceptr_t)a.queue, (int)(blocks * ns_used), 1, p.stream) != hipSuccess) return VP_ERR_HIP;
     const dim3 grid((unsigned)blocks), block(64 * VP_FITG2_WAVES);
     if (uniform && !weighted) hipLaunchKernelGGL((fitg2_kernel<M, NS, true, false>), grid, block, 0, p.stream, a);
     else if (uniform) hipLaunchKernelGGL((fitg2_kernel<M, NS, true, true>), grid, block, 0, p.stream, a);
diff --git a/varpro_amd/csrc/vp_generic.hpp b/varpro_amd/csrc/vp_generic.hpp
--- a/varpro_amd/csrc/vp_generic.hpp
+++ b/varpro_amd/csrc/vp_generic.hpp
@@ -49,6 +49,9 @@
     int list_first;
     int scale_cols;
     int ws_lds;
+    T *alpha_user, *C_user;
+    vp_report *report_user;
+
 };
 #ifndef VP_GEN_LDS_KB
 #define VP_GEN_LDS_KB 150
@@ -675,6 +678,8 @@
                 rep.n_evals = S.nfev;
                 rep.objective = (double)S.objective;
                 for (int k = 0; k < QQ; ++k) a.alpha_io[b * q + k] = S.x[k];
+                if (a.alpha_user)
+                    for (int k = 0; k < QQ; ++k) a.alpha_user[b * q + k] = S.x[k];
                 if (a.status) a.status[b] = S.status;
             });
             if (q == 0) {
@@ -684,9 +689,12 @@
                 if (a.status) a.status[b] = VP_ST_NOT_EVALUATED;
             }
             a.report[b] = rep;
+            if (a.report_user) a.report_user[b] = rep;
             if (a.cost_out) a.cost_out[b] = rep.objective;
             if (a.C_out)
                 for (int k = 0; k < n; ++k) a.C_out[b * n + k] = cbest[k];
+            if (a.C_user)
+                for (int k = 0; k < n; ++k) a.C_user[b * n + k] = cbest[k];
         }
         __syncthreads();
     }
@@ -1090,6 +1098,9 @@
     a.S = p.S > 0 ? p.S : 1;
     a.alpha = (const T *)p.alpha;
     a.alpha_io = (T *)p.alpha_out;
+    a.alpha_user = p.gen_list ? (T *)p.alpha_user : nullptr;
+    a.C_user = p.gen_list ? (T *)p.C_user : nullptr;
+    a.report_user = p.gen_list ? p.report_user : nullptr;
     a.r_out = (T *)p.r_out;
     a.J_out = (T *)p.J_out;
     a.C_out = (T *)p.C_out;
diff --git a/varpro_amd/csrc/vp_kernels.hpp b/varpro_amd/csrc/vp_kernels.hpp
--- a/varpro_amd/csrc/vp_kernels.hpp
+++ b/varpro_amd/csrc/vp_kernels.hpp
@@ -28,6 +28,11 @@
     const void *yw;
     const void *alpha;
     void *alpha_out;
+    const void *alpha_in;
+    void *alpha_user;
+    void *C_user;
+    vp_report *report_user;
+    int *io_direct;
     void *r_out;
     void *J_out;
     void *C_out;
```

After: 31.53 million fits/s. About the same (-0.2%).
